# chenkovsky/aha

Measured on AMD Instinct MI355X. Metric: input GB/s scanned + M-hits/s, 100k-pattern AC over 1 GiB UTF-8 corpus, higher is better.
Workload: dtype u8

## Files before the change

aha_amd/csrc/image.hpp:

```cpp
#pragma once
#include <cstdint>

#include "../../include/aha_hip.h"

namespace aha {

struct DevAut {
  const void *slots;
  const int32_t *end_key;
  const uint32_t *end_info;
  const uint2 *key_ln;
  const uint32_t *key_cnt;
  const uint32_t *key_kc;
  const uint32_t *key_info;
  const uint2 *chain;
  const uint2 *chain_chars;
  uint32_t root;
  uint32_t n_slots;
  uint32_t max_len;
  uint32_t compact;
  uint32_t s1_lo;
  uint32_t s2_lo;
  uint32_t s2_hi;
  const uint32_t *stale_bits;
  const uint32_t *term_bits;
};

struct MatchArgs {
  const uint8_t *text;
  const uint64_t *doc_off;
  uint64_t n_docs;
  uint64_t n_bytes;
  uint64_t n_chunks;
  uint32_t chunk;
  int32_t chars;
  int32_t sep;
  uint32_t sep_block[8];
  int32_t has_nul;
  int32_t no_filter;
  int32_t no_pair;
  int32_t check_docs;
  uint32_t *counts;
  uint32_t *leads;
  uint64_t *blk_hits;
  uint64_t *blk_leads;
  uint64_t *docg;
  uint64_t *totals;
  aha_hit *out;
  uint64_t cap;
  uint64_t *doc_hit_off;
  int32_t count_only;
  unsigned long long *kc_visits;
  unsigned long long *kc_hits;
  unsigned long long *kc_out;
  int32_t neutral;
  uint32_t *cover_mask;
  uint64_t cover_bit0;
  int32_t cover_clear;
  int32_t fold;
};

constexpr int kBlock = 256;

constexpr int kV2Threads = 1024;
constexpr int kV2Piece = 32;
constexpr uint32_t kV2Slab = 512;
constexpr uint32_t kV2MaxS = 32768;

struct V2Args {
  const uint8_t *text;
  const uint64_t *doc_off;
  uint64_t n_docs;
  uint64_t n_bytes;
  uint64_t n_chunks;
  uint32_t S;
  uint32_t lds_slots;
  int32_t chars;
  int32_t sep;
  uint32_t sep_block[8];
  uint4 *ev;
  uint32_t *ev_aux;
  uint64_t ev_cap;
  unsigned long long *cursor;
  uint32_t *slab_used;
  uint32_t *ev_cnt;
  uint32_t *lead_cnt;
  uint32_t *chunk_doc0;
  uint32_t *doc_ev_rank;
  uint32_t *doc_lead_rank;
  uint64_t *ev_base;
  uint64_t *lead_base;
  uint64_t *blk_a;
  uint64_t *blk_b;
  uint4 *sorted_ev;
  uint32_t *sorted_aux;
  uint32_t *sorted_cnt;
  uint64_t *totals;
  int32_t direct;
  int32_t dense_hits;
  uint32_t ev_stride;
  uint2 *evd;
  uint32_t *evg;
  uint32_t *doc_hit_rank;
  uint32_t unit_bb;
  uint32_t *chunk_hits;
  uint64_t *hit_base;
  aha_hit *out;
  uint64_t cap;
  uint64_t *doc_hit_off;
  unsigned long long *publish;
  unsigned long long *clear_next;
  uint32_t doc_from, doc_lanes16;
};

struct UnitDev {
  const uint2 *slots;
  const uint32_t *root;
  const uint32_t *tables;
  uint32_t n_slots;
  uint32_t big_lo;
  uint32_t n_low;
  uint32_t g0;
  uint32_t base_bits;
  uint32_t n_syms;
  uint32_t max_len;
  uint32_t hdr_beside;
};
size_t unit_lds_bytes(uint32_t n_syms);
int unit_prepare(uint32_t n_syms);
void unit_launch_traverse(const UnitDev &U, const V2Args &M, uint32_t grid, void *stream);
void unit_launch_regroup(const DevAut &A, const V2Args &M, void *stream);
void unit_launch_expand(const uint2 *uend, const DevAut &A, const V2Args &M, uint32_t workgroups, void *stream);
void v2_launch_hit_scan(const V2Args &M, void *stream);
void v2_launch_lead_scan(const V2Args &M, void *stream);

struct SkipDev {
  const uint32_t *bloom;
  uint32_t log2;
  uint32_t k1;
};
int skip_prepare(uint32_t n_syms, uint32_t log2_words);
size_t skip_bitmap_bytes(uint64_t n_bytes);
void skip_launch_mark(const SkipDev &K, const V2Args &M, void *bitmap, uint32_t grid, void *stream);
void skip_launch_traverse(const UnitDev &U, const V2Args &M, const void *bitmap, uint32_t grid, void *stream);

struct PairDev {
  const uint32_t *bloom;
  const uint4 *tab;
  const uint8_t *disp;
  uint32_t bloom_log2, k1, log2, groups;
};

int pair_prepare(uint32_t n_syms, uint32_t bloom_log2, uint32_t groups);
uint32_t pair_tile_bytes();
size_t pair_cand_bytes(uint64_t cap);
size_t pair_walk_bytes(uint64_t cap);
void pair_launch(const PairDev &P, const UnitDev &U, const DevAut &A, const V2Args &M, void *tile_dn, void *cand, void *wres,
                 uint64_t cand_cap, uint32_t grid, void *mid_event, void *stream);

constexpr uint32_t kFilterMul = 0x9E3779B1u;
constexpr uint32_t kFilterLog2 = 14;
struct FilterDev {
  const uint32_t *bloom;
  uint32_t d;
  uint32_t log2;
};
bool filter_image_in_lds(uint32_t n_slots, uint32_t chunk_bytes, bool chars = false);
int filter_prepare();
size_t filter_chunk_rec_bytes();
void filter_launch_filter(const FilterDev &F, const V2Args &M, void *bitmap, void *chunk_rec, unsigned long long *non_ascii,
                          uint32_t cus, void *stream);
void filter_launch_walk(const DevAut &A, const V2Args &M, const void *bitmap, const void *chunk_rec, const unsigned long long *non_ascii,
                        uint32_t cus, void *stream);

void filter_launch_filter_fold(const FilterDev &F, const V2Args &M, void *bitmap, void *chunk_rec, unsigned long long *non_ascii,
                               uint32_t cus, void *stream);
void filter_launch_walk_fold(const DevAut &A, const V2Args &M, const void *bitmap, const void *chunk_rec,
                             const unsigned long long *non_ascii, uint32_t cus, void *stream);
void fold_launch_copy(const uint8_t *src, uint8_t *dst, uint64_t n_bytes, uint32_t max_blocks, void *stream);
void fold2_launch_copy(const uint8_t *src, uint8_t *dst, uint64_t n_bytes, const uint64_t *doc_offsets, uint64_t n_docs,
                       uint32_t max_blocks, void *stream);
void fold3_launch_copy(const uint8_t *src, uint8_t *dst, uint64_t n_bytes, const uint64_t *doc_offsets, uint64_t n_docs,
                       uint32_t max_blocks, void *stream);
void fold3_launch_fix(const uint8_t *src, uint8_t *dst, uint64_t n_bytes, const uint64_t *doc_offsets, uint64_t n_docs,
                      uint32_t max_blocks, void *stream);
uint32_t fold_grid(uint64_t n_bytes, uint32_t max_blocks);
void foldk_launch_copy(const uint8_t *src, uint8_t *dst, uint64_t n_bytes, const uint64_t *doc_offsets, uint64_t n_docs,
                       uint32_t max_blocks, void *stream);

size_t v2_lds_bytes(uint32_t lds_slots, bool compact);
int v2_prepare(bool compact, size_t lds_bytes);
void v2_launch_traverse(const DevAut &A, const V2Args &M, uint32_t grid, void *stream);
void v2_launch_chunk_scan(const V2Args &M, void *stream);
void v2_launch_sort(const DevAut &A, const V2Args &M, uint64_t n_records, void *stream);
void v2_launch_expand(const DevAut &A, const V2Args &M, uint64_t n_events, void *stream);
void v2_launch_direct_post(const DevAut &A, const V2Args &M, void *stream, void *ev_mid, bool counted = false);
void v2_launch_count_post(const DevAut &A, const V2Args &M, void *stream, bool counted);
void v2_launch_doc_offsets(const DevAut &A, const V2Args &M, void *stream);
void unit_launch_doc_offsets(const V2Args &M, void *stream);
void count_launch_visits(const DevAut &A, const V2Args &M, const uint2 *uend, unsigned long long *visits, uint32_t max_blocks,
                         void *stream);
void count_launch_chain(const uint2 *key_ln, uint32_t n_keys, const unsigned long long *visits, unsigned long long *out,
                        const unsigned long long *abortf, void *stream);

void cover_launch_clear(uint32_t *words, uint64_t n_words, const unsigned long long *abortf, uint32_t max_blocks, void *stream);
void cover_launch_spans(const DevAut &A, const V2Args &M, const uint2 *uend, uint64_t *cdoc, uint32_t *mask, uint64_t bit0,
                        uint32_t max_blocks, void *stream);
void cover_launch_redact(const uint8_t *src, uint8_t *dst, const uint32_t *mask, uint64_t n_bytes, uint8_t fill, uint32_t max_blocks,
                         void *stream);
void cover_launch_doc_covered(const uint32_t *mask, const uint64_t *doc_off, uint64_t n_docs, uint64_t *doc_covered,
                              uint32_t max_blocks, void *stream);
void cover_launch_total(const uint32_t *mask, uint64_t n_words, uint64_t *total, uint32_t max_blocks, void *stream);

struct DcItem {
  uint64_t begin;
  uint32_t *out;
  uint32_t n;
  uint32_t doc;
};
constexpr uint32_t kDcSortMax = 4096;
constexpr uint32_t kDcRangeKeys = 8192;
constexpr uint32_t kDcSliceHits = 1u << 16;
void doccount_launch_sort(const DcItem *items, uint32_t n_items, const void *hits, uint32_t *n_pairs, void *stream);
void doccount_launch_range(const DcItem *items, uint32_t n_items, const void *hits, uint32_t n_keys, uint32_t range_keys,
                           uint32_t *n_pairs, void *stream);
void doccount_launch_add(const DcItem *slices, uint32_t n_slices, const void *hits, uint32_t *rows, uint32_t n_keys,
                         uint32_t max_blocks, void *stream);
void doccount_launch_compact(const DcItem *docs, uint32_t n_rows, uint32_t *rows, uint32_t n_keys, uint32_t *n_pairs, void *stream);
void doccount_launch_compact64(const DcItem *doc, unsigned long long *row, uint32_t n_keys, uint32_t *n_pairs, void *stream);
void doccount_launch_gather(const uint64_t *pair_off, const uint32_t *const *src, uint64_t n_docs, uint64_t n, void *out,
                            void *stream);

uint64_t select_rank_blocks(uint64_t n_bytes);
void select_launch_longest(const void *hits, uint64_t n_hits, const uint64_t *hit_off, const uint64_t *rel, uint64_t nd, uint64_t nb,
                           uint64_t *L, uint32_t max_blocks, void *stream);
void select_launch_marks(const uint64_t *L, uint64_t nb, const uint64_t *rel, uint64_t nd, uint32_t *cover, uint32_t *doc_start,
                         uint32_t max_blocks, void *stream);
void select_launch_walk(const uint64_t *L, uint64_t nb, const uint32_t *cover, const uint32_t *doc_start, uint32_t *select,
                        uint32_t max_blocks, void *stream);
void select_launch_rank(const uint32_t *select, uint64_t nb, uint64_t *blk, uint32_t max_blocks, void *stream);
void select_launch_rank_docs(const uint32_t *select, const uint64_t *blk, const uint64_t *rel, uint64_t nd, uint64_t base,
                             uint64_t *out, uint32_t max_blocks, void *stream);
void select_launch_emit(const uint32_t *select, uint64_t nb, const uint64_t *blk, const uint64_t *L, const uint64_t *rel, uint64_t nd,
                        void *out, uint32_t max_blocks, void *stream);

void tokens_launch_spans(const uint64_t *L, uint64_t nb, const uint32_t *select, uint32_t *S, uint32_t max_blocks, void *stream);
void tokens_launch_starts(const uint8_t *text, uint64_t nb, const uint32_t *select, const uint32_t *S, const uint32_t *doc_start,
                          bool gap_runs, uint32_t *T, uint32_t max_blocks, void *stream);
void tokens_launch_emit(const uint32_t *T, uint64_t nb, const uint64_t *blk, const uint32_t *select, const uint32_t *doc_start,
                        const uint64_t *L, const uint64_t *rel, uint64_t nd, void *out, uint32_t max_blocks, void *stream);

struct RepEntry {
  uint64_t off;
  uint32_t len;
  uint32_t keep;
};
constexpr uint32_t kRpScanBlock = 256;
inline uint64_t replace_scan_blocks(uint64_t n) { return (n + kRpScanBlock - 1) / kRpScanBlock; }
void replace_launch_delta(const void *sel, uint64_t n, const uint64_t *dso, const uint64_t *doc_off, uint64_t n_docs,
                          const RepEntry *ent, uint32_t n_keys, uint64_t *start, int64_t *shift, uint32_t max_blocks, void *stream);
void replace_launch_scan(int64_t *shift, uint64_t n, int64_t *sums, uint32_t max_blocks, void *stream);
void replace_launch_doc_offsets(const uint64_t *doc_off, const uint64_t *dso, const int64_t *shift, uint64_t n_docs,
                                uint64_t *doc_out, uint32_t max_blocks, void *stream);
void replace_launch_copy(const uint8_t *text, const void *sel, const uint64_t *start, const int64_t *shift, uint64_t n,
                         const RepEntry *ent, uint32_t n_keys, const uint8_t *blob, uint8_t *out, uint64_t total,
                         uint32_t max_blocks, void *stream);

void grep_launch_ends(const uint8_t *corpus, uint64_t n_bytes, uint8_t delim, const uint64_t *doc_off, uint64_t n_docs, uint32_t *mask,
                      uint32_t max_blocks, void *stream);
void grep_launch_emit_ends(const uint32_t *mask, uint64_t n_bytes, const uint64_t *blk, uint64_t *rec_off, uint32_t max_blocks,
                           void *stream);
void grep_launch_flag(const uint64_t *dho, uint64_t n_docs, bool invert, uint32_t *keep, uint32_t *S, uint32_t *T, uint32_t max_blocks,
                      void *stream);
void grep_launch_runs(const uint32_t *S, const uint32_t *T, uint64_t n_docs, const uint64_t *blk_s, const uint64_t *blk_t,
                      const uint64_t *doc_off, uint64_t n_runs, uint64_t *start, int64_t *shift, void *sel, RepEntry *ent,
                      uint32_t max_blocks, void *stream);
void grep_launch_emit_docs(const uint32_t *keep, const uint32_t *S, uint64_t n_docs, const uint64_t *blk_k, const uint64_t *blk_s,
                           const uint64_t *doc_off, const int64_t *shift, uint64_t n_runs, uint64_t *kept_docs, uint64_t *doc_out,
                           uint32_t max_blocks, void *stream);

void excerpt_launch_edges(const uint32_t *M, uint64_t n_bytes, const uint64_t *doc_off, uint64_t n_docs, uint32_t *S, uint32_t *T,
                          uint32_t max_blocks, void *stream);
void excerpt_launch_windows(const uint32_t *S, const uint32_t *T, uint64_t n_bytes, const uint64_t *blk_s, const uint64_t *blk_t,
                            const uint8_t *corpus, const uint64_t *doc_off, uint64_t n_docs, uint32_t before, uint32_t after,
                            uint64_t n_runs, uint64_t *doc, uint64_t *w0, uint64_t *w1, uint32_t *first, uint32_t *last,
                            uint32_t max_blocks, void *stream);
void excerpt_launch_gaps(const uint32_t *first, const uint32_t *last, uint64_t n_runs, const uint64_t *blk_f, const uint64_t *blk_l,
                         const uint64_t *w0, const uint64_t *w1, uint64_t n_bytes, uint64_t n_exc, uint64_t *start, int64_t *shift,
                         void *sel, RepEntry *ent, uint32_t max_blocks, void *stream);
void excerpt_launch_emit(const uint64_t *start, const int64_t *shift, uint64_t n_exc, uint64_t *starts, uint64_t *out_off,
                         uint32_t max_blocks, void *stream);

constexpr uint32_t kRuleMaxTerms = 64;
constexpr uint32_t kRuleChunkClasses = 32;
void greprule_launch_keep(const uint32_t *rows, uint32_t n_classes, const uint64_t *doc_off, uint64_t n_docs,
                          const aha_rule_term *terms, uint32_t n_terms, bool invert, uint32_t *keep, uint32_t max_blocks, void *stream);
void greprule_launch_edges(const uint32_t *keep, uint64_t n_docs, uint32_t *S, uint32_t *T, uint32_t max_blocks, void *stream);

constexpr uint32_t kCcSlice = 2048;
constexpr uint32_t kCcTable = 8192;
void classcount_launch_add(const void *hits, uint64_t n_hits, const uint64_t *hit_off, uint64_t nd, const uint64_t *cls_off,
                           const uint32_t *cls_ids, uint32_t n_keys, uint32_t n_classes, uint32_t *out, uint32_t max_blocks,
                           void *stream);
void classcount_launch_fold_keys(const uint64_t *key_counts, uint32_t n_keys, const uint64_t *cls_off, const uint32_t *cls_ids,
                                 uint32_t *row, uint32_t max_blocks, void *stream);

void launch_hits_pack(const int32_t *hits, uint64_t n, int32_t *pairs, void *stream);
void launch_hits_unpack(const DevAut &A, const int32_t *pairs, uint64_t n, int chars, int32_t *hits, void *stream);
struct StreamFmt {
  uint32_t step_bits;
  uint32_t len_bits;
};
void launch_hits_pack4(const int32_t *hits, uint64_t n, uint32_t *stream_words, unsigned long long *n_words, StreamFmt F,
                       void *stream);
void launch_hits_unpack4(const DevAut &A, const uint32_t *stream_words, uint64_t n, int chars, int32_t *hits, StreamFmt F,
                         void *stream);
constexpr uint32_t kMaxSegs = 64;
void launch_hits_unpack4_segs(const DevAut &A, const uint32_t *land, const uint64_t *word_off, const uint64_t *n_hits,
                              const uint64_t *out_off, uint32_t n_segs, int chars, int32_t *hits, StreamFmt F, void *stream);

void launch_publish_words(const unsigned long long *src, unsigned long long *host_dst, int n, void *stream);
void launch_check_docs(const uint64_t *doc_off, uint64_t n_docs, uint64_t n_bytes, uint32_t *flag, unsigned long long *abort_word,
                       void *stream);

void launch_count(const DevAut &A, const MatchArgs &M, void *stream);
void launch_scan_blocks(const MatchArgs &M, uint64_t n_blocks, void *stream);
void launch_count_doc_offsets(const MatchArgs &M, void *stream);
void launch_docg(const MatchArgs &M, void *stream);
void launch_write(const DevAut &A, const MatchArgs &M, void *stream);
void launch_has_nul(const uint8_t *text, uint64_t n, uint64_t *flag, void *stream);
void launch_longest(const DevAut &A, const MatchArgs &M, int mode, bool write, void *stream);

}
```

aha_amd/csrc/scan_unit.hip:

```cpp
#include <hip/hip_runtime.h>

#include "automaton.hpp"
#include "devcommon.hpp"
#include "image.hpp"
#include "unit.hpp"

namespace aha {

namespace {

constexpr int kUPiece = 16;
constexpr int kUWin = 3 * kUPiece;
constexpr int kURow = kUWin + 4;
constexpr int kUWave = 64 * kURow;

__device__ __forceinline__ uint4 load16(const uint8_t *text, int64_t g, int64_t N) {
  uint4 v = make_uint4(0, 0, 0, 0);
  if (g >= 0 && g + 16 <= N) {
    v = *reinterpret_cast<const uint4 *>(text + g);
  } else if (g >= 0 && g < N) {
    uint32_t w0 = 0, w1 = 0, w2 = 0, w3 = 0;
#pragma unroll 1
    for (int j = 0; j < 16 && g + j < N; j++) {
      const uint32_t b = (uint32_t)text[g + j] << ((j & 3) * 8);
      w0 |= (j >> 2) == 0 ? b : 0u;
      w1 |= (j >> 2) == 1 ? b : 0u;
      w2 |= (j >> 2) == 2 ? b : 0u;
      w3 |= (j >> 2) == 3 ? b : 0u;
    }
    v = make_uint4(w0, w1, w2, w3);
  }
  return v;
}

__device__ __forceinline__ uint64_t wballot(bool p) { return __builtin_amdgcn_ballot_w64(p); }
__device__ __forceinline__ bool wany(bool p) { return __builtin_amdgcn_ballot_w64(p) != 0ull; }
__device__ __forceinline__ bool wall(bool p) { return __builtin_amdgcn_ballot_w64(!p) == 0ull; }

__host__ __device__ inline size_t u_lds_rows(uint32_t n_syms) {
  return (size_t)(kUTabWords + ((n_syms + 3u) & ~3u)) * 4 + (size_t)(kV2Threads / 64) * kUWave + 16;
}
__host__ __device__ inline size_t u_lds_prog(uint32_t n_syms) {
  return u_lds_rows(n_syms) + (size_t)(kV2Threads / 64) * 64 * 12;
}
__host__ __device__ inline size_t u_lds(uint32_t n_syms) {
  return u_lds_prog(n_syms) + (size_t)(kV2Threads / 64) * 4;
}

template <bool CHARS, int BB, bool HB>
__global__ __launch_bounds__(kV2Threads) void ku_traverse(UnitDev U, V2Args M) {
  extern __shared__ __attribute__((aligned(16))) uint8_t smem[];
  if (M.cursor[1] >= 16ull) return;
  uint32_t *tabw = reinterpret_cast<uint32_t *>(smem);
  uint32_t *rlw = tabw + kUTabWords;
  const uint32_t n_root = (U.n_syms + 3u) & ~3u;
  for (uint32_t i = threadIdx.x; i < kUTabWords; i += kV2Threads) tabw[i] = U.tables[i];
  for (uint32_t i = threadIdx.x; i < n_root; i += kV2Threads) rlw[i] = i < U.n_syms ? U.root[i] : 0u;
  uint32_t *prog = reinterpret_cast<uint32_t *>(smem + u_lds_prog(U.n_syms));
  if (threadIdx.x < kV2Threads / 64) prog[threadIdx.x] = 0u;
  __syncthreads();
  const uint32_t *rl = rlw;
  const uint4 *t0a = reinterpret_cast<const uint4 *>(tabw + kUT0a);
  const uint2 *t0b = reinterpret_cast<const uint2 *>(tabw + kUT0b);
  const uint8_t *tabb = reinterpret_cast<const uint8_t *>(tabw);
  uint8_t *in_base = smem + (size_t)(kUTabWords + n_root) * 4;
  const int lane = threadIdx.x & 63, wave = threadIdx.x >> 6;
  uint8_t *inl = in_base + wave * kUWave + lane * kURow;
  const uint32_t *row = reinterpret_cast<const uint32_t *>(inl);
  typedef uint32_t v3u __attribute__((ext_vector_type(3)));
  const uint32_t wbo = (uint32_t)u_lds_rows(U.n_syms) + (uint32_t)wave * (64u * 12u);
  const uint2 *slots = U.slots;
  const int64_t N = (int64_t)M.n_bytes;
  const uint64_t D = M.n_docs;
  const int64_t S = (int64_t)M.S;
  const int rounds = (int)(M.S / kUPiece);
  const int warm = U.max_len > 1 ? (int)U.max_len - 1 : 0;
  const int R = (warm + kUPiece - 1) / kUPiece;
  const uint32_t wave_u = (uint32_t)__builtin_amdgcn_readfirstlane(wave);
  uint32_t *my_prog = prog + (wave_u & 3u) * 4u + (wave_u >> 2);
  const uint4 *simd_prog = reinterpret_cast<const uint4 *>(prog + (wave_u & 3u) * 4u);
  uint32_t n_rounds = 0;

  const uint64_t n_tiles = (M.n_chunks + kV2Threads - 1) / kV2Threads;
  for (uint64_t tile = blockIdx.x; tile < n_tiles; tile += gridDim.x) {
    const uint64_t chunk = tile * kV2Threads + threadIdx.x;
    const uint32_t ev_stride = M.ev_stride;
    const bool live = chunk < M.n_chunks;
    const int64_t a = (int64_t)chunk * S;
    const int64_t e = live ? min(a + S, N) : a;
    uint64_t dn = 0;
    int64_t nb = INT64_MAX, doc_start = a, pos = e;
    uint32_t wfill = 0, wout = 0;
    const uint64_t wchunk0 = tile * kV2Threads + (uint64_t)wave * 64;
    uint32_t *wreg = M.evg + wchunk0 * M.ev_stride * 3;
    const uint32_t wcap = (uint32_t)min<uint64_t>(64, M.n_chunks > wchunk0 ? M.n_chunks - wchunk0 : 0) * M.ev_stride;
    uint32_t hits = 0;
    uint32_t lead_total = 0;
    uint32_t lc = 0, lc_exact = 0;
    uint32_t E = 0, seq = 0;
    uint32_t pc = 0;
    uint4 q1 = make_uint4(0, 0, 0, 0), q2 = q1, q3 = q1;
    uint32_t w[13] = {0, 0, 0, 0, 0, 0, 0, 0, 0, 0, 0, 0, 0};
    if (live) {
      dn = first_boundary(M.doc_off, D, (uint64_t)a);
      nb = (int64_t)M.doc_off[dn];
      pos = a;
      if (nb != a) {
        doc_start = (int64_t)M.doc_off[dn - 1];
        pos = a - min<int64_t>(a - doc_start, warm);
        if (CHARS) M.chunk_doc0[chunk] = (uint32_t)(dn - 1);
      } else if (CHARS) {
        M.chunk_doc0[chunk] = (uint32_t)dn;
      }
    }

    for (int r = -((R + 3) / 4) * 4 - 2; r <= rounds; r++) {
      {
        n_rounds++;
        if (lane == 0) *my_prog = n_rounds;
        const uint4 pm = *simd_prog;
        const uint32_t ahead = ((uint32_t)__builtin_amdgcn_readfirstlane(pm.x) > n_rounds) + ((uint32_t)__builtin_amdgcn_readfirstlane(pm.y) > n_rounds) +
                               ((uint32_t)__builtin_amdgcn_readfirstlane(pm.z) > n_rounds) + ((uint32_t)__builtin_amdgcn_readfirstlane(pm.w) > n_rounds);
        if (ahead == 0u)
          __builtin_amdgcn_s_setprio(0);
        else if (ahead == 1u)
          __builtin_amdgcn_s_setprio(1);
        else if (ahead == 2u)
          __builtin_amdgcn_s_setprio(2);
        else
          __builtin_amdgcn_s_setprio(3);
      }
      const int64_t pb = a + (int64_t)r * kUPiece;
      const int64_t pl = pb + 2 * kUPiece;
      const int64_t pend = min(pb + kUWin, e);
      {
        uint4 v;
        if ((pl & 63) == 0) {
          v = load16(M.text, pl, N);
          q1 = load16(M.text, pl + 16, N);
          q2 = load16(M.text, pl + 32, N);
          q3 = load16(M.text, pl + 48, N);
        } else {
          v = q1;
          q1 = q2;
          q2 = q3;
        }
#pragma unroll
        for (int i = 0; i < 9; i++) w[i] = w[i + 4];
        w[9] = v.x;
        w[10] = v.y;
        w[11] = v.z;
        w[12] = v.w;
        uint32_t *dst = reinterpret_cast<uint32_t *>(inl);
#pragma unroll
        for (int i = 0; i < 13; i++) dst[i] = w[i];
      }
      const bool need = live && pos < pend;
      if (!wany(need)) continue;
      uint32_t rel = kURow, lim = 0;
      if (need) {
        rel = (uint32_t)(pos - pb + 4);
        lim = (uint32_t)(pend - pb + 4);
      }
      uint32_t nb_rel = (nb >= pb - 4 && nb <= pb + kUWin) ? (uint32_t)(nb - pb + 4) : ~0u;
      const uint32_t n_rel = (N - pb) <= (int64_t)kUWin ? (uint32_t)max<int64_t>(N - pb + 4, 0) : ~0u;
      const int32_t a_rel = (int32_t)max<int64_t>(a - pb + 4, -128);
      const int32_t e_rel = (int32_t)min<int64_t>(e - pb + 4, 128);
      int32_t docrel = (int32_t)(pb - 4 - doc_start);

      for (;;) {
        const bool bnd = rel < lim && rel == nb_rel;
        if (wany(bnd)) {
          if (bnd) {
            const int64_t here = pb - 4 + rel;
            do {
              M.doc_ev_rank[dn] = seq;
              M.doc_hit_rank[dn] = hits;
              if (CHARS) M.doc_lead_rank[dn] = lead_total;
              dn++;
              nb = dn <= D ? (int64_t)M.doc_off[dn] : INT64_MAX;
            } while (nb == here);
            asm volatile("" : "+v"(nb));
            nb_rel = (nb <= pb + kUWin) ? (uint32_t)(nb - pb + 4) : ~0u;
            E = 0;
            pc = 0;
            lc = 0;
            lc_exact = 1;
            doc_start = here;
            docrel = -(int32_t)rel;
          }
        }
        uint32_t lim2 = min(lim, nb_rel);
        const uint32_t dend = min(nb_rel, n_rel);
        auto decode = [&](uint32_t at, uint32_t &o_code, uint32_t &o_L, bool &o_later) {
          const uint32_t lo = row[at >> 2], hi = row[(at >> 2) + 1];
          const uint32_t w4 = __builtin_amdgcn_alignbyte(hi, lo, at & 3u);
          const uint32_t b0 = w4 & 0xFFu;
          const uint4 q0 = t0a[b0];
          const uint2 q1 = t0b[b0];
          const uint32_t s1 = *reinterpret_cast<const uint32_t *>(tabb + q0.x + ((w4 >> 6) & 0x3FCu));
          const uint32_t s2 = *reinterpret_cast<const uint32_t *>(tabb + q0.y + ((w4 >> 14) & 0x3FCu));
          const uint32_t sum = q0.z + s1 + s2;
          const uint32_t want = q1.y;
          const bool in_doc = at + want <= dend;
          o_later = in_doc & at + want > (uint32_t)kURow;
          const bool whole = in_doc & sum < kUPoison;
          const bool o_good = whole & (sum - q0.w) < q1.x;
          o_L = whole ? want : 1u;
          if (CHARS) o_L |= (b0 & 0xC0u) != 0x80u ? 0x100u : 0u;
          o_code = o_good ? sum - kUBias : 0u;
        };
        uint32_t code, L;
        {
          bool later;
          decode(min(rel, (uint32_t)kURow), code, L, later);
          lim2 = later ? min(lim2, rel) : lim2;
          lim = later ? min(lim, rel) : lim;
        }
        bool all_left = false;
        for (;;) {
          const bool act = rel < lim2;
          all_left = wall(rel >= (uint32_t)(4 + kUPiece) || rel >= lim);
          if (all_left || !wany(act)) break;
          auto trip = [&]() -> uint32_t {
            uint32_t evc = 0;
            const bool good = code != 0u;
            const uint32_t Bq = u_child(E, BB);
            const bool hdr = u_hdr_pending(E);
            const bool grp = Bq >= U.big_lo & code >= U.n_low & !hdr;
            uint32_t se = grp ? (code >> 5) + U.g0 : code;
            se = hdr ? 0u : se;
            const uint32_t fc = BB == 22 ? (code & 7u) : min(code & 7u, 6u);
            const bool probe = act & good & (((E | 0x20000000u) >> ((uint32_t)BB + fc)) & 1u) != 0u & Bq != 0u;
            unsigned long long enw = 0;
            uint32_t hdw = 0;
            {
              const uint2 *ap = slots + (probe ? (Bq ^ se) : 0u);
              asm volatile("global_load_dwordx2 %0, %1, off" : "=v"(enw) : "v"(ap) : "memory");
              if (HB) {
                const uint2 *hp = slots + ((act & u_nfr(E) & !u_f1(E)) ? Bq : 0u);
                asm volatile("global_load_dword %0, %1, off" : "=v"(hdw) : "v"(hp) : "memory");
              }
            }
            if (act) {
              uint32_t n_code, n_L;
              bool n_later;
              const uint32_t Lb = CHARS ? (L & 0xFFu) : L;
              uint32_t rel_adv = rel + Lb;
              decode(rel_adv, n_code, n_L, n_later);
              const uint32_t rt = rl[code];
              const uint32_t rf = rl[pc];
              const bool viaroot0 = !u_nfr(E) | !good;
              const bool own0 = viaroot0 | u_f1(E);
              const uint32_t ft0 = u_f1(E) ? (rf & 0x7FFFFFFFu) : (Bq | u_all_filter(BB) | 0x20000000u);
              uint32_t miss0 = viaroot0 ? rt : (HB ? (rf & 0x7FFFFFFFu) : ft0);
              const uint32_t cb = code & 31u;
              uint32_t lowm = ~(~0u << cb);
              uint32_t gbit = (grp & probe) ? (1u << cb) : 0u;
              const bool pg = probe & !grp;
              const bool pgh = pg & !hdr;
              const int32_t last = (int32_t)rel_adv - 1;
              uint32_t wm = (last >= a_rel & last < e_rel) ? ~0u : 0u;
              uint32_t isl0 = (CHARS && (int32_t)rel >= a_rel) ? (L >> 8) : 0u;
              if (CHARS) asm volatile("" : "+v"(isl0));
              if (HB)
                asm volatile("s_waitcnt vmcnt(0)" : "+v"(enw), "+v"(hdw), "+v"(miss0), "+v"(rel_adv), "+v"(lowm), "+v"(gbit), "+v"(wm), "+v"(n_code), "+v"(n_L) : : "memory");
              else
                asm volatile("s_waitcnt vmcnt(0)" : "+v"(enw), "+v"(miss0), "+v"(rel_adv), "+v"(lowm), "+v"(gbit), "+v"(wm), "+v"(n_code), "+v"(n_L) : : "memory");
              const uint32_t enx = (uint32_t)enw, eny = (uint32_t)(enw >> 32);
              const bool symeq = u_sym(eny) == se;
              const bool symhit = symeq & pg;
              const bool hit = symeq & pgh;
              const bool redir = (enx & gbit) != 0u;
              const uint32_t rE = (__builtin_popcount(enx & lowm) + eny ^ code) | u_all_filter(BB);
              const bool viaroot = !(symhit | redir) & viaroot0;
              uint32_t missE = HB ? (own0 ? miss0 : hdw) : miss0;
              missE = redir ? rE : missE;
              E = symhit ? enx : missE;
              const bool consumed = hit | viaroot;
              const bool end = consumed & u_end(E);
              const uint32_t c4 = hit ? u_c4(eny) : 1u;
              pc = consumed ? code : pc;
              if (CHARS) {
                const uint32_t isl = consumed ? isl0 : 0u;
                lc += isl;
                lead_total += isl;
              }
              rel = consumed ? rel_adv : rel;
              const bool park = consumed & n_later;
              lim2 = park ? rel : lim2;
              lim = park ? rel : lim;
              code = consumed ? n_code : code;
              L = consumed ? n_L : L;
              evc = end ? (c4 & wm) : 0u;
            }
            return evc;
          };
          const uint32_t evc = trip();
          const uint64_t evm = wballot(evc != 0u);
          if (evm) {
            const bool ev = evc != 0u;
            const uint32_t kp = __popcll(evm);
            if (wfill + kp > 64u) {
              const uint32_t *q = reinterpret_cast<const uint32_t *>(smem + (wbo + __umul24((uint32_t)lane, 12u)));
              const v3u r = {q[0], q[1], q[2]};
              if ((uint32_t)lane < wfill && wout + (uint32_t)lane < wcap) *reinterpret_cast<v3u *>(wreg + (size_t)(wout + lane) * 3) = r;
              wout += wfill;
              wfill = 0;
            }
            const uint32_t my = wfill + __builtin_amdgcn_mbcnt_hi((uint32_t)(evm >> 32), __builtin_amdgcn_mbcnt_lo((uint32_t)evm, 0u));
            const uint32_t rx = u_rec_x(u_child(E, BB), (uint32_t)lane, evc, BB), rz = u_rec_z(hits, evc, BB);
            const uint32_t ry = CHARS ? ((lc << 1) | lc_exact) : (uint32_t)(docrel + (int32_t)rel);
            if (ev) {
              uint32_t *d = reinterpret_cast<uint32_t *>(smem + (wbo + __umul24(my, 12u)));
              d[0] = rx;
              d[1] = ry;
              d[2] = rz;
            }
            wfill += kp;
            seq += ev ? 1u : 0u;
            hits += evc;
          }
        }
        if (all_left || !wany(rel < lim)) break;
      }
      if (need) pos = pb - 4 + rel;
    }
    {
      const uint32_t *q = reinterpret_cast<const uint32_t *>(smem + (wbo + __umul24((uint32_t)lane, 12u)));
      const v3u r = {q[0], q[1], q[2]};
      if ((uint32_t)lane < wfill && wout + (uint32_t)lane < wcap) *reinterpret_cast<v3u *>(wreg + (size_t)(wout + lane) * 3) = r;
    }
    if (live) {
      M.ev_cnt[chunk] = seq;
      if (seq > ev_stride) M.cursor[1] = 2ull;
      if (CHARS) M.lead_cnt[chunk] = lead_total;
      M.chunk_hits[chunk] = hits;
      if (e == N) {
        while (dn <= D) {
          M.doc_ev_rank[dn] = seq;
          M.doc_hit_rank[dn] = hits;
          if (CHARS) M.doc_lead_rank[dn] = lead_total;
          dn++;
        }
      }
    }
  }
}

constexpr int kRgThreads = 256, kRgPer = 4, kRgBlock = kRgThreads * kRgPer, kRgSubs = kRgBlock / 64;
__global__ __launch_bounds__(kRgThreads) void ku_regroup(DevAut A, V2Args M) {
  __shared__ uint2 s_sorted[kRgBlock];
  __shared__ uint8_t s_lane[kRgBlock];
  __shared__ uint32_t s_cnt[kRgSubs][64], s_part[kRgThreads / 64][64];
  __shared__ uint32_t s_start[64], s_tot[64], s_run[64], s_hits[64];
  if (M.cursor[1]) return;
  const int lane = threadIdx.x & 63, wv = threadIdx.x >> 6;
  const uint64_t n_groups = (M.n_chunks + 63) / 64;
  const uint32_t stride = M.ev_stride;
  const uint32_t bb = M.unit_bb, bmask = (1u << bb) - 1u;
  for (uint64_t g = blockIdx.x; g < n_groups; g += gridDim.x) {
    __syncthreads();
    if (wv == 0) {
      s_run[lane] = 0;
      s_hits[lane] = 0;
    }
    const uint64_t c = g * 64 + lane;
    uint32_t total = c < M.n_chunks ? min(M.ev_cnt[c], stride) : 0u;
#pragma unroll
    for (int d = 32; d >= 1; d >>= 1) total += __shfl_xor(total, d, 64);
    const uint32_t *src = M.evg + g * 64 * stride * 3;
    uint2 *dst = M.evd + g * 64 * stride;
    uint2 nxt[kRgPer];
    uint32_t xn[kRgPer];
#pragma unroll
    for (int q = 0; q < kRgPer; q++) {
      const uint32_t i = q * kRgThreads + threadIdx.x;
      nxt[q] = i < total ? make_uint2(src[(size_t)i * 3], src[(size_t)i * 3 + 1]) : make_uint2(0, 0);
    }
#pragma unroll
    for (int q = 0; q < kRgPer; q++) xn[q] = (uint32_t)(q * kRgThreads) + threadIdx.x < total ? A.end_info[nxt[q].x & bmask] : 0u;
    for (uint32_t i0 = 0; i0 < total; i0 += kRgBlock) {
      uint2 rec[kRgPer];
      uint32_t x[kRgPer], rank[kRgPer], l[kRgPer];
      bool live[kRgPer];
#pragma unroll
      for (int q = 0; q < kRgPer; q++) {
        const uint32_t i = i0 + q * kRgThreads + threadIdx.x;
        live[q] = i < total;
        rec[q] = nxt[q];
        x[q] = xn[q];
        nxt[q] = i + kRgBlock < total ? make_uint2(src[(size_t)(i + kRgBlock) * 3], src[(size_t)(i + kRgBlock) * 3 + 1])
                                      : make_uint2(0, 0);
      }
#pragma unroll
      for (int q = 0; q < kRgPer; q++) {
        l[q] = (rec[q].x >> bb) & 63u;
        uint64_t same = __ballot(live[q]), mine = same;
#pragma unroll
        for (int b = 0; b < 6; b++) {
          const uint64_t bal = __ballot(live[q] & ((l[q] >> b) & 1u) != 0u);
          same &= ((l[q] >> b) & 1u) ? bal : ~bal;
          mine &= ((lane >> b) & 1) ? bal : ~bal;
        }
        rank[q] = __popcll(same & ((1ull << lane) - 1ull));
        s_cnt[q * (kRgThreads / 64) + wv][lane] = __popcll(mine);
      }
      __syncthreads();
      {
        uint32_t acc = 0;
#pragma unroll
        for (int r = 0; r < kRgSubs / (kRgThreads / 64); r++) {
          const uint32_t v = s_cnt[wv * (kRgSubs / (kRgThreads / 64)) + r][lane];
          s_cnt[wv * (kRgSubs / (kRgThreads / 64)) + r][lane] = acc;
          acc += v;
        }
        s_part[wv][lane] = acc;
      }
      __syncthreads();
      if (wv == 0) {
        uint32_t acc = 0;
#pragma unroll
        for (int w2 = 0; w2 < kRgThreads / 64; w2++) {
          const uint32_t v = s_part[w2][lane];
          s_part[w2][lane] = acc;
          acc += v;
        }
        s_tot[lane] = acc;
        s_start[lane] = wave_incl_scan(acc) - acc;
      }
      __syncthreads();
#pragma unroll
      for (int q = 0; q < kRgPer; q++) {
        if (live[q]) {
          const uint32_t sb = q * (kRgThreads / 64) + wv;
          const uint32_t p = s_start[l[q]] + s_part[sb / (kRgSubs / (kRgThreads / 64))][l[q]] + s_cnt[sb][l[q]] + rank[q];
          uint32_t cnt = x[q] >> 24;
          if (cnt == 255u) cnt = A.key_cnt[A.chain ? A.chain[x[q] & 0xFFFFFFu].y : (x[q] & 0xFFFFFFu)];
          s_sorted[p] = make_uint2(x[q], rec[q].y);
          s_lane[p] = (uint8_t)l[q];
          if (cnt) atomicAdd(&s_hits[l[q]], cnt);
        }
      }
      __syncthreads();
#pragma unroll
      for (int q = 0; q < kRgPer; q++)
        xn[q] = i0 + kRgBlock + (uint32_t)(q * kRgThreads) + threadIdx.x < total ? A.end_info[nxt[q].x & bmask] : 0u;
#pragma unroll
      for (int q = 0; q < kRgPer; q++) asm volatile("" : "+v"(xn[q]));
      const uint32_t nb = min(total - i0, (uint32_t)kRgBlock);
#pragma unroll
      for (int q = 0; q < kRgPer; q++) {
        const uint32_t p = q * kRgThreads + threadIdx.x;
        if (p < nb) {
          const uint32_t lp = s_lane[p];
          const uint32_t at = s_run[lp] + (p - s_start[lp]);
          if (at < stride) dst[(uint64_t)lp * stride + at] = s_sorted[p];
        }
      }
      __syncthreads();
      if (wv == 0) s_run[lane] += s_tot[lane];
    }
    __syncthreads();
    if (wv == 0 && c < M.n_chunks) M.chunk_hits[c] = s_hits[lane];
  }
}

constexpr int kXgThreads = 1024, kXgPer = 1, kXgBlock = kXgThreads * kXgPer, kXgStage = 1536;
constexpr int kXgCacheBits = 11;
template <bool CHARS>
__global__ __launch_bounds__(kXgThreads) void ku_expand_groups(const uint2 *uend, DevAut A, V2Args M) {
  __shared__ uint32_t s_hs[kXgStage], s_he[kXgStage], s_hk[kXgStage];
  __shared__ uint8_t s_hl[kXgStage];
  __shared__ uint32_t s_tot[2][64], s_start[64], s_run[64], s_all;
  __shared__ uint64_t s_base[64];
  __shared__ uint32_t s_adj[64];
  __shared__ unsigned long long s_cache[1 << kXgCacheBits];
  if (M.cursor[1]) return;
  const int lane = threadIdx.x & 63, wv = threadIdx.x >> 6;
  const uint64_t n_groups = (M.n_chunks + 63) / 64;
  const uint32_t stride = M.ev_stride;
  const uint32_t bb = M.unit_bb, bmask = (1u << bb) - 1u;
  for (uint32_t i = threadIdx.x; i < (1u << kXgCacheBits); i += kXgThreads) s_cache[i] = 0ull;
  for (uint64_t g = blockIdx.x; g < n_groups; g += gridDim.x) {
    __syncthreads();
    const uint64_t c = g * 64 + lane;
    if (wv == 0) {
      if (CHARS && c < M.n_chunks) s_adj[lane] = M.lead_cnt[c];
      s_base[lane] = c < M.n_chunks ? M.hit_base[c] : 0ull;
      s_run[lane] = 0;
      s_tot[0][lane] = 0;
    }
    uint32_t total = c < M.n_chunks ? min(M.ev_cnt[c], stride) : 0u;
#pragma unroll
    for (int d = 32; d >= 1; d >>= 1) total += __shfl_xor(total, d, 64);
    const uint32_t *src = M.evg + g * 64 * stride * 3;
    typedef uint32_t v3u __attribute__((ext_vector_type(3)));
    v3u nxt[kXgPer];
#pragma unroll
    for (int q = 0; q < kXgPer; q++) {
      const uint32_t i = q * kXgThreads + threadIdx.x;
      nxt[q] = i < total ? __builtin_nontemporal_load(reinterpret_cast<const v3u *>(src + (size_t)i * 3)) : v3u{0, 0, 0};
    }
    __syncthreads();
    uint32_t par = 0;
    for (uint32_t i0 = 0; i0 < total; i0 += kXgBlock, par ^= 1u) {
      v3u rec[kXgPer];
      uint2 ue[kXgPer];
      bool live[kXgPer], keep[kXgPer];
      uint32_t cs[kXgPer];
#pragma unroll
      for (int q = 0; q < kXgPer; q++) {
        const uint32_t i = i0 + q * kXgThreads + threadIdx.x;
        live[q] = i < total;
        rec[q] = nxt[q];
        nxt[q] = i + kXgBlock < total ? __builtin_nontemporal_load(reinterpret_cast<const v3u *>(src + (size_t)(i + kXgBlock) * 3)) : v3u{0, 0, 0};
        const uint32_t b = rec[q].x & bmask, n = u_rec_n(rec[q].x, rec[q].z, bb);
        cs[q] = (b * 0x9E3779B1u) >> (32 - kXgCacheBits);
        const unsigned long long ce = s_cache[cs[q]];
        const bool cached = live[q] & n == 1u & (uint32_t)ce == b + 1u;
        ue[q] = make_uint2((uint32_t)(ce >> 32), 0u);
        if (live[q] && !cached) ue[q] = uend[b];
        keep[q] = live[q] & !cached & n == 1u;
        if (live[q]) atomicAdd(&s_tot[par][(rec[q].x >> bb) & 63u], n);
      }
      __syncthreads();
      if (wv == 0) {
        const uint32_t t = s_tot[par][lane];
        const uint32_t incl = wave_incl_scan(t);
        s_start[lane] = incl - t;
        if (lane == 63) s_all = incl;
        s_tot[par ^ 1u][lane] = 0;
      }
      __syncthreads();
      const uint32_t T = s_all;
#pragma unroll
      for (int q = 0; q < kXgPer; q++)
        if (keep[q] && (ue[q].y >> 24) == 0u)
          atomicExch(&s_cache[cs[q]], (unsigned long long)ue[q].x << 32 | ((rec[q].x & bmask) + 1u));
      for (uint32_t w0 = 0; w0 < T; w0 += kXgStage) {
#pragma unroll
        for (int q = 0; q < kXgPer; q++) {
          if (live[q]) {
            const uint32_t l = (rec[q].x >> bb) & 63u, n = u_rec_n(rec[q].x, rec[q].z, bb);
            const uint32_t pos = s_start[l] + (u_rec_before(rec[q].z) - s_run[l]);
            const uint32_t end = CHARS ? (rec[q].y >> 1) + ((rec[q].y & 1u) ? 0u : s_adj[l]) : rec[q].y, co = ue[q].y & 0xFFFFFFu;
            uint32_t len = (ue[q].x >> 24) | (ue[q].y >> 24) << 8, key = ue[q].x & 0xFFFFFFu;
            for (uint32_t k = 0;;) {
              const uint32_t j = pos + k - w0;
              if (j < (uint32_t)kXgStage) {
                s_hs[j] = end - len;
                s_he[j] = end;
                s_hk[j] = key;
                s_hl[j] = (uint8_t)l;
              }
              if (++k >= n) break;
              const uint2 ce = (CHARS ? A.chain_chars : A.chain)[co + k];
              len = ce.x;
              key = ce.y;
            }
          }
        }
        __syncthreads();
        const uint32_t nh = min(T - w0, (uint32_t)kXgStage);
        for (uint32_t j = threadIdx.x; j < nh; j += kXgThreads) {
          const uint32_t l = s_hl[j];
          const uint64_t idx = s_base[l] + s_run[l] + (w0 + j - s_start[l]);
          if (idx < M.cap) {
            aha_hit hit;
            hit.start = (int32_t)s_hs[j];
            hit.end = (int32_t)s_he[j];
            hit.value = (int32_t)s_hk[j];
            M.out[idx] = hit;
          }
        }
        __syncthreads();
      }
      if (wv == 0) s_run[lane] += s_tot[par][lane];
    }
  }
}

__global__ __launch_bounds__(256) void ku_chunk_adj(V2Args M) {
  if (M.cursor[1]) return;
  const uint64_t c = (uint64_t)blockIdx.x * 256 + threadIdx.x;
  if (c >= M.n_chunks) return;
  const uint32_t d0 = M.chunk_doc0[c];
  const uint64_t dchunk = M.doc_off[d0] / M.S;
  M.lead_cnt[c] = (uint32_t)(M.lead_base[c] - (M.lead_base[dchunk] + M.doc_lead_rank[d0]));
}

__global__ __launch_bounds__(256) void ku_doc_offsets(V2Args M) {
  if (M.publish && blockIdx.x == 0 && threadIdx.x < 5) M.publish[threadIdx.x] = M.cursor[threadIdx.x];
  if (M.clear_next && blockIdx.x == 0 && threadIdx.x < 16) M.clear_next[threadIdx.x] = 0ull;
  if (M.cursor[1] || !M.doc_hit_off) return;
  const uint64_t d = (uint64_t)blockIdx.x * 256 + threadIdx.x;
  if (d > M.n_docs) return;
  const uint64_t q = M.doc_off[d];
  M.doc_hit_off[d] = q < M.n_bytes ? M.hit_base[q / M.S] + M.doc_hit_rank[d] : M.totals[0];
}

}

size_t unit_lds_bytes(uint32_t n_syms) { return u_lds(n_syms); }

int unit_prepare(uint32_t n_syms) {
  const int lds = (int)unit_lds_bytes(n_syms);
  int e = 0;
#define AHA_PREP_KU(C, B, H) \
  if (!e) e = (int)hipFuncSetAttribute((const void *)ku_traverse<C, B, H>, hipFuncAttributeMaxDynamicSharedMemorySize, lds);
  AHA_PREP_KU(false, 22, false) AHA_PREP_KU(true, 22, false) AHA_PREP_KU(false, 23, false) AHA_PREP_KU(true, 23, false)
  AHA_PREP_KU(false, 22, true) AHA_PREP_KU(true, 22, true) AHA_PREP_KU(false, 23, true) AHA_PREP_KU(true, 23, true)
#undef AHA_PREP_KU
  return e;
}

void unit_launch_traverse(const UnitDev &U, const V2Args &M, uint32_t grid, void *stream) {
  const size_t lds = unit_lds_bytes(U.n_syms);
#define AHA_LAUNCH_KU(C, B, H) hipLaunchKernelGGL((ku_traverse<C, B, H>), dim3(grid), dim3(kV2Threads), lds, (hipStream_t)stream, U, M)
#define AHA_LAUNCH_KU2(C, B) \
  do {                       \
    if (U.hdr_beside)        \
      AHA_LAUNCH_KU(C, B, true);  \
    else                     \
      AHA_LAUNCH_KU(C, B, false); \
  } while (0)
  if (U.base_bits == 23) {
    if (M.chars) AHA_LAUNCH_KU2(true, 23); else AHA_LAUNCH_KU2(false, 23);
  } else {
    if (M.chars) AHA_LAUNCH_KU2(true, 22); else AHA_LAUNCH_KU2(false, 22);
  }
#undef AHA_LAUNCH_KU2
#undef AHA_LAUNCH_KU
}

void unit_launch_doc_offsets(const V2Args &M, void *stream) {
  if (M.doc_hit_off)
    hipLaunchKernelGGL(ku_doc_offsets, dim3((uint32_t)((M.n_docs + 1 + 255) / 256)), dim3(256), 0, (hipStream_t)stream, M);
}

void unit_launch_regroup(const DevAut &A, const V2Args &M, void *stream) {
  const uint64_t n_groups = (M.n_chunks + 63) / 64;
  hipLaunchKernelGGL(ku_regroup, dim3((uint32_t)std::min<uint64_t>(n_groups, 1u << 16)), dim3(kRgThreads), 0,
                     (hipStream_t)stream, A, M);
}

void unit_launch_expand(const uint2 *uend, const DevAut &A, const V2Args &M, uint32_t workgroups, void *stream) {
  const uint64_t n_groups = (M.n_chunks + 63) / 64;
  const dim3 grid((uint32_t)std::max<uint64_t>(1, std::min<uint64_t>(n_groups, workgroups)));
  if (M.chars) {
    hipLaunchKernelGGL(ku_chunk_adj, dim3((uint32_t)((M.n_chunks + 255) / 256)), dim3(256), 0, (hipStream_t)stream, M);
    hipLaunchKernelGGL(ku_expand_groups<true>, grid, dim3(kXgThreads), 0, (hipStream_t)stream, uend, A, M);
  } else {
    hipLaunchKernelGGL(ku_expand_groups<false>, grid, dim3(kXgThreads), 0, (hipStream_t)stream, uend, A, M);
  }
  if (M.doc_hit_off)
    hipLaunchKernelGGL(ku_doc_offsets, dim3((uint32_t)((M.n_docs + 1 + 255) / 256)), dim3(256), 0, (hipStream_t)stream, M);
}

}
```

aha_amd/csrc/unit.cpp:

```cpp
#include "unit.hpp"

#include <algorithm>
#include <cstdio>
#include <cstdlib>
#include <cstring>
#include <chrono>

namespace aha {

namespace {

struct UTrans {
  uint32_t sym;
  uint32_t child;
  uint32_t raw;
};

}

static void build_unit_bits(const Automaton &a, UnitImage &u, bool force, uint32_t base_bits) {
  u = UnitImage();
  u.base_bits = base_bits;
  const uint32_t max_slots = 1u << base_bits;
  const uint32_t S = a.n_states;
  if (a.n_keys == 0 || S < 2) {
    u.why = "no keys";
    return;
  }
  if (a.n_keys > (1u << 24)) {
    u.why = "more than 2^24 keys";
    return;
  }
  std::vector<uint8_t> need(S, 0);
  for (uint32_t s = 0; s < S; s++) {
    for (uint32_t j = 0; j < a.n_child[s]; j++) {
      const uint32_t c = a.first_child[s] + j;
      const uint32_t b = a.in_label[c];
      if (need[s]) {
        if ((b & 0xC0u) != 0x80u) {
          u.why = "a key holds a lead byte without its continuation bytes";
          return;
        }
        need[c] = (uint8_t)(need[s] - 1);
      } else if (b < 0x80u) {
        need[c] = 0;
      } else if ((b & 0xE0u) == 0xC0u) {
        need[c] = 1;
      } else if ((b & 0xF0u) == 0xE0u) {
        need[c] = 2;
      } else {
        u.why = "a key holds a stray continuation byte or a byte >= 0xF0";
        return;
      }
    }
    if (a.key_of[s] >= 0 && need[s]) {
      u.why = "a key ends inside a unit";
      return;
    }
  }
  for (uint32_t s = 1; s < S; s++)
    if (need[s] == 0 && need[a.fail[s]] != 0) {
      u.why = "a fail link leaves the unit boundaries";
      return;
    }
  uint64_t multi = 0, all = 0;
  for (uint32_t s = 1; s < S; s++) {
    all++;
    if (a.in_label[s] >= 0x80u) multi++;
  }
  u.multi_permille = (uint32_t)(multi * 1000 / std::max<uint64_t>(all, 1));
  if (!force && u.multi_permille < 300) {
    u.why = "fewer than 30 % of the key bytes lie in multi-byte units";
    return;
  }

  std::vector<uint32_t> first(S + 1, 0);
  std::vector<UTrans> tr;
  tr.reserve(S);
  std::vector<uint32_t> ustates;
  uint32_t lo2 = ~0u, hi2 = 0, lo3 = ~0u, hi3 = 0;
  for (uint32_t s = 0; s < S; s++) {
    first[s] = (uint32_t)tr.size();
    if (need[s]) continue;
    ustates.push_back(s);
    for (uint32_t j = 0; j < a.n_child[s]; j++) {
      const uint32_t c1 = a.first_child[s] + j;
      const uint32_t b0 = a.in_label[c1];
      if (need[c1] == 0) {
        tr.push_back({(1u << 16) | b0, c1, b0});
        continue;
      }
      for (uint32_t j2 = 0; j2 < a.n_child[c1]; j2++) {
        const uint32_t c2 = a.first_child[c1] + j2;
        const uint32_t b1 = a.in_label[c2];
        if (need[c2] == 0) {
          const uint32_t p = ((b0 & 0x1Fu) << 6) | (b1 & 0x3Fu);
          lo2 = std::min(lo2, p);
          hi2 = std::max(hi2, p + 1);
          tr.push_back({(2u << 16) | p, c2, b0 | b1 << 8});
          continue;
        }
        for (uint32_t j3 = 0; j3 < a.n_child[c2]; j3++) {
          const uint32_t c3 = a.first_child[c2] + j3;
          const uint32_t b2 = a.in_label[c3];
          const uint32_t p = ((b0 & 0x0Fu) << 12) | ((b1 & 0x3Fu) << 6) | (b2 & 0x3Fu);
          lo3 = std::min(lo3, p);
          hi3 = std::max(hi3, p + 1);
          tr.push_back({(3u << 16) | p, c3, b0 | b1 << 8 | b2 << 16});
        }
      }
    }
  }
  first[S] = (uint32_t)tr.size();
  u.n_states = (uint32_t)ustates.size();
  u.n_trans = (uint32_t)tr.size();
  if (getenv("AHA_DEBUG")) fprintf(stderr, "aha: unit image: %u states, %u transitions, %u-bit bases\n", u.n_states, u.n_trans, base_bits);
  if ((uint64_t)u.n_states + u.n_states / 8 + 1 > max_slots) {
    u.why = "more states than the bases address";
    return;
  }

  u.c2lo = hi2 ? lo2 : 0;
  u.w2 = hi2 ? hi2 - lo2 : 0;
  u.c3lo = hi3 ? lo3 : 0;
  u.w3 = hi3 ? hi3 - lo3 : 0;
  u.n1 = 128;
  u.n2 = 129 + u.w2;
  u.n_syms = u.n2 + 1 + u.w3;
  if (u.n_syms > kUMaxSyms) {
    u.why = "the keys' characters span more symbols than the root table holds in LDS";
    return;
  }
  for (UTrans &t : tr) {
    const uint32_t cls = t.sym >> 16, p = t.sym & 0xFFFFu;
    t.sym = cls == 1 ? p : (cls == 2 ? 129 + (p - u.c2lo) : u.n2 + 1 + (p - u.c3lo));
  }
  for (uint32_t s : ustates)
    if (!std::is_sorted(tr.begin() + first[s], tr.begin() + first[s + 1], [](const UTrans &x, const UTrans &y) { return x.sym < y.sym; }))
      std::sort(tr.begin() + first[s], tr.begin() + first[s + 1], [](const UTrans &x, const UTrans &y) { return x.sym < y.sym; });
  u.tables.assign(kUTabWords, 0u);
  for (uint32_t b = 0; b < 256; b++) {
    uint32_t a1 = 0, a2 = 0, L = 1, lo = 1, span = 127;
    int64_t base = 0;
    if (b >= 1 && b < 0x80) {
      base = b;
    } else if ((b & 0xE0u) == 0xC0u) {
      L = 2;
      a1 = (kUA1 + 256) * 4;
      lo = 129;
      span = u.w2;
      base = 129 + (int64_t)((b & 0x1Fu) << 6) - u.c2lo;
    } else if ((b & 0xF0u) == 0xE0u) {
      L = 3;
      a1 = (kUA1 + 512) * 4;
      a2 = (kUA2 + 256) * 4;
      lo = u.n2 + 1;
      span = u.w3;
      base = (int64_t)u.n2 + 1 + (int64_t)((b & 0x0Fu) << 12) - u.c3lo;
    }
    if (L == 1) {
      a1 = kUA1 * 4;
      a2 = kUA2 * 4;
    } else if (L == 2) {
      a2 = kUA2 * 4;
    }
    u.tables[kUT0a + 4 * b + 0] = a1;
    u.tables[kUT0a + 4 * b + 1] = a2;
    u.tables[kUT0a + 4 * b + 2] = (uint32_t)(base + kUBias);
    u.tables[kUT0a + 4 * b + 3] = lo + kUBias;
    u.tables[kUT0b + 2 * b + 0] = span;
    u.tables[kUT0b + 2 * b + 1] = L;
    const bool cont = (b & 0xC0u) == 0x80u;
    u.tables[kUA1 + 256 + b] = cont ? (b & 0x3Fu) : kUPoison;
    u.tables[kUA1 + 512 + b] = cont ? ((b & 0x3Fu) << 6) : kUPoison;
    u.tables[kUA2 + 256 + b] = cont ? (b & 0x3Fu) : kUPoison;
  }

  std::vector<uint8_t> udepth(S, 0);
  for (uint32_t s : ustates)
    for (uint32_t t = first[s]; t < first[s + 1]; t++) udepth[tr[t].child] = (uint8_t)std::min<uint32_t>(udepth[s] + 1u, 255u);
  for (uint32_t s : ustates)
    if (udepth[s] == 1 && a.key_of[s] >= 0) u.unit_key = true;
  {
    std::vector<uint8_t> de(S, 0);
    for (uint32_t s : ustates)
      for (uint32_t t = first[s]; t < first[s + 1]; t++) {
        const uint32_t c = tr[t].child;
        de[c] = (uint8_t)std::min<uint32_t>(de[s] + ((udepth[c] >= 3 && a.key_of[c] >= 0) ? 1u : 0u), 255u);
        u.deep_ends_max = std::max<uint32_t>(u.deep_ends_max, de[c]);
      }
  }
  if (!u.unit_key) {
    struct Pair {
      uint32_t raw0, raw1, child, h;
    };
    std::vector<Pair> pairs;
    for (uint32_t t0 = first[0]; t0 < first[1]; t0++) {
      const uint32_t c0 = tr[t0].child;
      for (uint32_t t1 = first[c0]; t1 < first[c0 + 1]; t1++) pairs.push_back({tr[t0].raw, tr[t1].raw, tr[t1].child, 0u});
    }
    u.n_pairs = (uint32_t)pairs.size();
    static const uint32_t k1s[] = {kSkipKA, 0xC2B2AFu, 0x27D4EBu, 0x165667u, 0xD3A264u, 0xFD7047u, 0xB55A4Fu, 0x7FEB35u};
    bool placed = false;
    for (uint32_t k1 : k1s) {
      if (pairs.empty() || pairs.size() > (size_t)kPairMaxGroups * 8) break;
      for (Pair &p : pairs) p.h = sk_hash(sk_part(p.raw0), p.raw1, k1);
      std::vector<uint32_t> sorted(pairs.size());
      for (size_t i = 0; i < pairs.size(); i++) sorted[i] = pairs[i].h;
      std::sort(sorted.begin(), sorted.end());
      if (std::adjacent_find(sorted.begin(), sorted.end()) != sorted.end()) continue;
      uint32_t G = 256;
      while (G < kPairMaxGroups && G * 4u < pairs.size()) G <<= 1;
      std::vector<std::vector<uint32_t>> groups(G);
      for (uint32_t i = 0; i < pairs.size(); i++) groups[pt_group(pairs[i].h, G)].push_back(i);
      std::vector<uint32_t> order(G);
      for (uint32_t g = 0; g < G; g++) order[g] = g;
      std::stable_sort(order.begin(), order.end(), [&](uint32_t x, uint32_t y) { return groups[x].size() > groups[y].size(); });
      uint32_t lg = 8;
      while (((size_t)1 << lg) * 2u < pairs.size() * 3u) lg++;
      for (; lg <= 21 && !placed; lg++) {
        std::vector<uint32_t> tab((size_t)4 << lg, 0u);
        std::vector<uint8_t> disp(G, 0);
        bool okp = true;
        std::vector<uint32_t> slots;
        for (uint32_t gi = 0; okp && gi < G; gi++) {
          const std::vector<uint32_t> &grp = groups[order[gi]];
          if (grp.empty()) break;
          uint32_t d = 0;
          for (; d < 256; d++) {
            slots.clear();
            bool fits = true;
            for (uint32_t i : grp) {
              const uint32_t sl = pt_slot(pairs[i].h, d, lg);
              if (tab[4 * (size_t)sl] != 0 || std::find(slots.begin(), slots.end(), sl) != slots.end()) {
                fits = false;
                break;
              }
              slots.push_back(sl);
            }
            if (fits) break;
          }
          if (d == 256) {
            okp = false;
            break;
          }
          disp[order[gi]] = (uint8_t)d;
          for (size_t j = 0; j < grp.size(); j++) {
            const Pair &p = pairs[grp[j]];
            uint32_t cf = 0;
            for (uint32_t t2 = first[p.child]; t2 < first[p.child + 1]; t2++) cf |= pt_cls(tr[t2].raw);
            const int32_t key = a.key_of[p.child];
            const uint32_t c4 = key >= 0 ? std::min<uint32_t>(a.key_cnt[key], kUMaxC4) : 0u;
            uint32_t *e = &tab[4 * (size_t)slots[j]];
            e[0] = p.raw0 | c4 << 24;
            e[1] = p.raw1;
            e[2] = (uint32_t)key;
            e[3] = cf;
          }
        }
        if (okp) {
          u.pair_tab.swap(tab);
          u.pair_disp.swap(disp);
          u.pair_log2 = lg;
          u.pair_groups = G;
          u.pair_k1 = k1;
          placed = true;
        }
      }
      if (placed) break;
    }
    if (!placed) {
      u.pair_k1 = kSkipKA;
      for (Pair &p : pairs) p.h = sk_hash(sk_part(p.raw0), p.raw1, u.pair_k1);
    }
    for (uint32_t lg = kSkipMinLog2; !pairs.empty() && lg <= kSkipMaxLog2; lg++) {
      u.mark_bloom.assign((size_t)1 << lg, 0u);
      for (const Pair &p : pairs) u.mark_bloom[sk_word(p.h, lg)] |= sk_mask(p.h);
      uint64_t bits = 0;
      for (uint32_t x : u.mark_bloom) bits += (uint64_t)__builtin_popcount(x);
      u.mark_log2 = lg;
      u.mark_fill_permille = (uint32_t)(bits * 1000 / ((uint64_t)32 << lg));
      if (bits * 16 <= ((uint64_t)32 << lg)) break;
    }
  }
  auto has_header = [&](uint32_t s) {
    return s != 0 && a.fail[s] != 0 && udepth[a.fail[s]] != 1;
  };

  u.n_low = std::min<uint32_t>((u.n2 + 1 + 31u) & ~31u, 512u);
  u.g0 = u.n_low - (u.n_low >> 5);
  const uint32_t n_groups = u.n_syms > u.n_low ? (u.n_syms - u.n_low + 31u) / 32u : 0u;
  uint32_t bb = 64;
  while (bb < u.n_low + n_groups) bb <<= 1;
  u.big_block = bb;
  constexpr uint32_t kBlk = 1u << 15;
  constexpr uint32_t kMaxBlocks = kUMaxSlots / kBlk;
  struct Bits {
    std::vector<uint64_t> w;
    explicit Bits(size_t n) : w((n + 63) / 64, 0ull) {}
    bool get(uint32_t i) const { return (w[i >> 6] >> (i & 63)) & 1ull; }
    void set(uint32_t i) { w[i >> 6] |= 1ull << (i & 63); }
  };
  Bits used(kUMaxSlots), isb(kUMaxSlots);
  std::vector<uint32_t> freec(kMaxBlocks, kBlk), curw(kMaxBlocks, 0);
  std::vector<uint32_t> idfree(kMaxBlocks, kBlk);
  std::vector<uint32_t> base(S, 0);
  used.set(0);
  isb.set(0);
  freec[0]--;
  idfree[0]--;
  uint32_t n_open = 1, n_big = 0, n_bases = 1;
  std::vector<uint32_t> order, bigs;
  for (uint32_t s : ustates) {
    if (s == 0) continue;
    const uint32_t deg = first[s + 1] - first[s];
    if (deg >= kUBigDegree) {
      bigs.push_back(s);
    } else if (deg + (has_header(s) ? 1u : 0u) > 0) {
      order.push_back(s);
    }
  }
  n_big = (uint32_t)bigs.size();
  auto nsym = [&](uint32_t s) { return first[s + 1] - first[s] + (has_header(s) ? 1u : 0u); };
  std::stable_sort(order.begin(), order.end(), [&](uint32_t x, uint32_t y) {
    const uint32_t cx = udepth[x] == 1 ? 0u : 1u, cy = udepth[y] == 1 ? 0u : 1u;
    if (cx != cy) return cx < cy;
    return nsym(x) > nsym(y);
  });
  auto open_block = [&]() -> bool {
    if ((uint64_t)(n_open + 1) * kBlk + (uint64_t)n_big * bb > max_slots) {
      if (getenv("AHA_DEBUG"))
        fprintf(stderr, "aha: unit image: %u blocks open, %u big states of %u slots, %u bases so far: no room for another block\n",
                n_open, n_big, bb, n_bases);
      return false;
    }
    n_open++;
    return true;
  };
  uint32_t sy[kUBigDegree + 1];
  auto try_block = [&](uint32_t blk, uint32_t k) -> uint32_t {
    const uint32_t fr = freec[blk];
    if (fr < k) return 0;
    uint64_t budget = fr;
    if ((double)fr * idfree[blk] / kBlk < 0.5) return 0;
    if (k > 1) {
      double p = (double)idfree[blk] / kBlk;
      const double fl = (double)fr / kBlk;
      for (uint32_t i = 1; i < k; i++) p *= fl;
      if (p * fr < 0.5) return 0;
      budget = std::min<uint64_t>(fr, (uint64_t)(4.0 / p) + 1024);
    }
    const uint32_t w0 = blk * (kBlk / 64), nw = kBlk / 64;
    uint32_t wi = curw[blk];
    for (uint32_t step = 0; step < nw && budget; step++, wi = wi + 1 < nw ? wi + 1 : 0) {
      uint64_t fw = ~used.w[w0 + wi];
      while (fw && budget) {
        const uint32_t f = ((w0 + wi) << 6) + (uint32_t)__builtin_ctzll(fw);
        fw &= fw - 1;
        budget--;
        const uint32_t cand = f ^ sy[0];
        if (cand == 0 || isb.get(cand)) continue;
        bool okc = true;
        for (uint32_t i = 1; okc && i < k; i++) okc = !used.get(cand ^ sy[i]);
        if (okc) {
          curw[blk] = wi;
          return cand;
        }
      }
    }
    return 0;
  };
  uint32_t lowest = 0;
  std::vector<uint32_t> dead(kMaxBlocks, ~0u);
  auto place = [&](uint32_t k) -> uint32_t {
    while (lowest < n_open && freec[lowest] == 0) lowest++;
    for (uint32_t blk = lowest;; blk++) {
      if (blk == n_open && !open_block()) return 0;
      if (k >= dead[blk]) continue;
      const uint32_t b = try_block(blk, k);
      if (!b && (k > 1 || (double)freec[blk] * idfree[blk] / kBlk < 8.0)) dead[blk] = k;
      if (b) {
        for (uint32_t i = 0; i < k; i++) used.set(b ^ sy[i]);
        freec[blk] -= k;
        isb.set(b);
        idfree[blk]--;
        n_bases++;
        return b;
      }
    }
  };
  std::vector<std::vector<uint32_t>> big_runs(n_big);
  auto place_runs = [&]() -> bool {
    uint32_t t = kBlk;
    for (uint32_t bi = 0; bi < n_big; bi++) {
      const uint32_t s = bigs[bi];
      big_runs[bi].assign(n_groups, 0u);
      for (uint32_t q = first[s]; q < first[s + 1];) {
        if (tr[q].sym < u.n_low) {
          q++;
          continue;
        }
        const uint32_t g = (tr[q].sym - u.n_low) >> 5;
        uint32_t q2 = q;
        while (q2 < first[s + 1] && ((tr[q2].sym - u.n_low) >> 5) == g) q2++;
        const uint32_t cnt = q2 - q;
        for (;; t++) {
          if (t + cnt > n_open * kBlk) {
            if (!open_block()) return false;
          }
          if ((t & (kBlk - 1)) + cnt > kBlk) {
            t = (t | (kBlk - 1));
            continue;
          }
          bool okr = true;
          for (uint32_t j = 0; okr && j < cnt; j++) okr = !used.get(t + j) && !isb.get((t + j) ^ tr[q + j].sym);
          if (okr) break;
        }
        for (uint32_t j = 0; j < cnt; j++) {
          used.set(t + j);
          if (!isb.get((t + j) ^ tr[q + j].sym)) {
            isb.set((t + j) ^ tr[q + j].sym);
            idfree[t / kBlk]--;
            n_bases++;
          }
        }
        freec[t / kBlk] -= cnt;
        big_runs[bi][g] = t;
        t += cnt;
        q = q2;
      }
    }
    return true;
  };
  bool runs_done = n_big == 0 || n_groups == 0;
  const auto t_place = std::chrono::steady_clock::now();
  auto lap = [&](const char *what) {
    if (getenv("AHA_DEBUG"))
      fprintf(stderr, "aha: unit image: %s at %.2f s, %u blocks\n", what,
              std::chrono::duration<double>(std::chrono::steady_clock::now() - t_place).count(), n_open);
  };
  for (size_t oi = 0; oi < order.size(); oi++) {
    const uint32_t s = order[oi];
    if (!runs_done && udepth[s] != 1) {
      if (!place_runs()) {
        u.why = "more transitions than the bases address";
        return;
      }
      runs_done = true;
    }
    uint32_t k = 0;
    for (uint32_t t = first[s]; t < first[s + 1]; t++) sy[k++] = tr[t].sym;
    if (has_header(s)) sy[k++] = 0u;
    const uint32_t b = place(k);
    if (!b) {
      u.why = "more transitions than the bases address";
      return;
    }
    base[s] = b;
  }
  if (!runs_done && !place_runs()) {
    u.why = "more transitions than the bases address";
    return;
  }
  lap("states with slots placed");
  {
    uint32_t n_ids = 0;
    for (uint32_t s : ustates)
      if (s != 0 && first[s + 1] == first[s] && !has_header(s)) n_ids++;
    while ((uint64_t)n_open * kBlk < (uint64_t)n_bases + n_ids + 1)
      if (!open_block()) {
        u.why = "more states than the bases address";
        return;
      }
    uint32_t idc = 1;
    for (uint32_t s : ustates) {
      if (s == 0 || first[s + 1] != first[s] || has_header(s)) continue;
      while (isb.get(idc)) idc++;
      base[s] = idc;
      isb.set(idc);
    }
  }
  const uint32_t n_shared = n_open * kBlk;
  const uint32_t n_slots = ((n_shared + n_big * bb) + kBlk - 1) & ~(kBlk - 1);
  for (uint32_t bi = 0; bi < n_big; bi++) base[bigs[bi]] = n_shared + bi * bb;

  auto word = [&](uint32_t st) -> uint32_t {
    uint32_t flt = 0;
    for (uint32_t q = first[st]; q < first[st + 1]; q++) flt |= 1u << (tr[q].sym & 7u);
    if (first[st + 1] - first[st] >= kUBigDegree) flt = 0xFFu;
    const bool nfr = a.fail[st] != 0, f1 = nfr && udepth[a.fail[st]] == 1;
    return base[st] | ((flt << base_bits) & u_all_filter(base_bits)) | (f1 ? (1u << 29) : 0u) | (nfr ? (1u << 30) : 0u) |
           (a.key_of[st] >= 0 ? 0x80000000u : 0u);
  };
  auto u_c4_of = [](const Automaton &au, uint32_t st) -> uint32_t {
    return au.key_of[st] >= 0 ? std::min<uint32_t>(au.key_cnt[au.key_of[st]], kUMaxC4) : 0u;
  };
  u.n_slots = n_slots;
  u.n_shared = n_shared;
  u.n_big = n_big;
  u.slots.assign(n_slots, 0ull);
  u.end_key.assign(n_slots, -1);
  u.root.assign(u.n_syms, 0u);
  std::vector<uint32_t> big_index(n_big ? S : 0, 0u);
  for (uint32_t bi = 0; bi < n_big; bi++) big_index[bigs[bi]] = bi;
  for (uint32_t s : ustates) {
    const uint32_t b = base[s];
    const bool big = s != 0 && first[s + 1] - first[s] >= kUBigDegree;
    if (has_header(s)) {
      u.slots[b] = (uint64_t)(word(a.fail[s]) & 0x7FFFFFFFu);
      u.n_nfr++;
    }
    if (a.key_of[s] >= 0) u.end_key[b] = a.key_of[s];
    for (uint32_t t = first[s]; t < first[s + 1]; t++) {
      const uint32_t c = tr[t].child, sym = tr[t].sym;
      const uint64_t entry = ((uint64_t)(sym | u_c4_of(a, c) << 16) << 32) | word(c);
      if (s == 0) {
        u.root[sym] = word(c);
      } else if (!big || sym < u.n_low) {
        u.slots[b ^ sym] = entry;
      } else {
        const uint32_t g = (sym - u.n_low) >> 5, run = big_runs[big_index[s]][g];
        uint64_t &rec = u.slots[b + u.n_low + g];
        const uint32_t bits = (uint32_t)rec, rank = (uint32_t)__builtin_popcount(bits);
        rec = ((uint64_t)run << 32) | (bits | 1u << ((sym - u.n_low) & 31u));
        u.slots[run + rank] = entry;
      }
    }
  }
  u.ok = true;
}

void build_unit(const Automaton &a, UnitImage &u, bool force) {
  const char *bw = getenv("AHA_UNIT_BASE_BITS");
  if (bw && strcmp(bw, "23") == 0) {
    build_unit_bits(a, u, force, 23u);
    return;
  }
  build_unit_bits(a, u, force, 22u);
  if (!u.ok && strstr(u.why, "bases address")) build_unit_bits(a, u, force, 23u);
}

}
```

aha_amd/csrc/unit.hpp:

```cpp
#pragma once

#include <cstdint>
#include <vector>

#include "automaton.hpp"

namespace aha {

constexpr uint32_t kUMaxSlots = 1u << 23;
constexpr uint32_t kUBigDegree = 48;
constexpr uint32_t kUMaxSyms = 21756;
constexpr uint32_t kUBias = 1u << 17;
constexpr uint32_t kUPoison = 1u << 24;
constexpr uint32_t kUT0a = 0, kUT0b = 1024, kUA1 = 1536, kUA2 = 2304, kUTabWords = 2816;

AHA_HD inline uint32_t u_child(uint32_t lo, uint32_t bb = 22u) { return lo & ((1u << bb) - 1u); }
AHA_HD inline uint32_t u_all_filter(uint32_t bb) { return ((1u << (29u - bb)) - 1u) << bb; }
constexpr uint32_t kUMaxC4 = 255u;
constexpr uint32_t kUFusedMaxChain = 15u;
AHA_HD inline uint32_t u_rec_x(uint32_t base, uint32_t lane, uint32_t n, uint32_t bb) {
  return base | lane << bb | (n & ((1u << (26u - bb)) - 1u)) << (bb + 6u);
}
AHA_HD inline uint32_t u_rec_z(uint32_t hits_before, uint32_t n, uint32_t bb) { return hits_before | (n >> (26u - bb)) << 27; }
AHA_HD inline uint32_t u_rec_n(uint32_t x, uint32_t z, uint32_t bb) { return (x >> (bb + 6u)) | (z >> 27) << (26u - bb); }
AHA_HD inline uint32_t u_rec_before(uint32_t z) { return z & 0x7FFFFFFu; }
AHA_HD inline bool u_f1(uint32_t lo) { return ((lo >> 29) & 1u) != 0; }
AHA_HD inline bool u_nfr(uint32_t lo) { return ((lo >> 30) & 1u) != 0; }
AHA_HD inline bool u_end(uint32_t lo) { return (lo >> 31) != 0; }
AHA_HD inline uint32_t u_sym(uint32_t hi) { return hi & 0xFFFFu; }
AHA_HD inline uint32_t u_c4(uint32_t hi) { return (hi >> 16) & 255u; }
AHA_HD inline bool u_hdr_pending(uint32_t lo) { return ((lo >> 29) & 3u) == 1u; }

constexpr uint32_t kSkipKA = 0x9E3779u, kSkipKB = 0x85EBCBu;
constexpr uint32_t kSkipMinLog2 = 10, kSkipMaxLog2 = 14;
AHA_HD inline uint32_t sk_mul24(uint32_t a, uint32_t b) { return (a & 0xFFFFFFu) * (b & 0xFFFFFFu); }
AHA_HD inline uint32_t sk_part(uint32_t c0) {
  const uint32_t g = sk_mul24(c0, kSkipKB);
  return (g >> 11) | (g << 21);
}
AHA_HD inline uint32_t sk_hash(uint32_t part, uint32_t c1, uint32_t k1 = kSkipKA) {
  const uint32_t h = sk_mul24(c1, k1) + part;
  return h ^ (h >> 16);
}
AHA_HD inline uint32_t sk_word(uint32_t h, uint32_t log2_words) { return h >> (32u - log2_words); }
AHA_HD inline uint32_t sk_mask(uint32_t h) { return (1u << (h & 31u)) | (1u << ((h >> 5) & 31u)); }

constexpr uint32_t kPairMix = 0x2545F491u, kPairKC = 0xC2B2AFu;
constexpr uint32_t kPairMaxGroups = 16384;
constexpr uint32_t kPairMaxDeepEnds = 3;
AHA_HD inline uint32_t pt_group(uint32_t h, uint32_t n_groups) { return (h >> 7) & (n_groups - 1u); }
AHA_HD inline uint32_t pt_slot(uint32_t h, uint32_t d, uint32_t log2_slots) {
  const uint32_t t = h * kPairMix;
  return ((t >> (32u - log2_slots)) + d * ((t << 1) | 1u)) & ((1u << log2_slots) - 1u);
}
AHA_HD inline uint32_t pt_cls(uint32_t raw) {
  const uint32_t g = sk_mul24(raw, kPairKC);
  return (1u << (g >> 27)) | (1u << ((g >> 22) & 31u));
}

struct UnitImage {
  bool ok = false;
  const char *why = "";
  uint32_t n_slots = 0;
  uint32_t n_shared = 0;
  uint32_t n_big = 0, big_block = 0;
  uint32_t n_low = 0, g0 = 0;
  uint32_t base_bits = 22;
  std::vector<uint64_t> slots;
  std::vector<int32_t> end_key;
  std::vector<uint32_t> root;
  std::vector<uint32_t> tables;
  uint32_t n_syms = 0;
  uint32_t n1 = 128, n2 = 0;
  uint32_t c2lo = 0, w2 = 0, c3lo = 0, w3 = 0;
  uint32_t n_states = 0, n_trans = 0, n_nfr = 0;
  uint32_t multi_permille = 0;
  std::vector<uint32_t> mark_bloom;
  uint32_t mark_log2 = 0;
  uint32_t n_pairs = 0;
  uint32_t mark_fill_permille = 0;
  bool unit_key = false;
  uint32_t pair_k1 = kSkipKA;
  std::vector<uint32_t> pair_tab;
  std::vector<uint8_t> pair_disp;
  uint32_t pair_log2 = 0, pair_groups = 0;
  uint32_t deep_ends_max = 0;
};

void build_unit(const Automaton &a, UnitImage &u, bool force = false);

}
```

Before: 494.8.

## Add 21-bit base encoding for unit automaton images with dedicated traverse kernel

Moves the traverse kernel into a shared header and adds a 21-bit-base variant, picked automatically when the slot table and identities fit in 2^21 and exceed a minimum size, unless skip/pair engines are opted in. Fewer base bits leave more filter bits in each state word (u_all_filter widens), so fewer transitions should need a global slot probe. The cost is extra build logic and another kernel instantiation. Correctness now depends on tracking the identity range accurately.

```diff
diff --git a/aha_amd/csrc/image.hpp b/aha_amd/csrc/image.hpp
--- a/aha_amd/csrc/image.hpp
+++ b/aha_amd/csrc/image.hpp
@@ -129,6 +129,8 @@
 size_t unit_lds_bytes(uint32_t n_syms);
 int unit_prepare(uint32_t n_syms);
 void unit_launch_traverse(const UnitDev &U, const V2Args &M, uint32_t grid, void *stream);
+int unit21_prepare(uint32_t n_syms);
+void unit21_launch_traverse(const UnitDev &U, const V2Args &M, uint32_t grid, void *stream);
 void unit_launch_regroup(const DevAut &A, const V2Args &M, void *stream);
 void unit_launch_expand(const uint2 *uend, const DevAut &A, const V2Args &M, uint32_t workgroups, void *stream);
 void v2_launch_hit_scan(const V2Args &M, void *stream);
diff --git a/aha_amd/csrc/scan_unit.hip b/aha_amd/csrc/scan_unit.hip
--- a/aha_amd/csrc/scan_unit.hip
+++ b/aha_amd/csrc/scan_unit.hip
@@ -1,352 +1,8 @@
-#include <hip/hip_runtime.h>
-
-#include "automaton.hpp"
-#include "devcommon.hpp"
-#include "image.hpp"
-#include "unit.hpp"
+#include "scan_unit_walk.hpp"
 
 namespace aha {
 
 namespace {
-
-constexpr int kUPiece = 16;
-constexpr int kUWin = 3 * kUPiece;
-constexpr int kURow = kUWin + 4;
-constexpr int kUWave = 64 * kURow;
-
-__device__ __forceinline__ uint4 load16(const uint8_t *text, int64_t g, int64_t N) {
-  uint4 v = make_uint4(0, 0, 0, 0);
-  if (g >= 0 && g + 16 <= N) {
-    v = *reinterpret_cast<const uint4 *>(text + g);
-  } else if (g >= 0 && g < N) {
-    uint32_t w0 = 0, w1 = 0, w2 = 0, w3 = 0;
-#pragma unroll 1
-    for (int j = 0; j < 16 && g + j < N; j++) {
-      const uint32_t b = (uint32_t)text[g + j] << ((j & 3) * 8);
-      w0 |= (j >> 2) == 0 ? b : 0u;
-      w1 |= (j >> 2) == 1 ? b : 0u;
-      w2 |= (j >> 2) == 2 ? b : 0u;
-      w3 |= (j >> 2) == 3 ? b : 0u;
-    }
-    v = make_uint4(w0, w1, w2, w3);
-  }
-  return v;
-}
-
-__device__ __forceinline__ uint64_t wballot(bool p) { return __builtin_amdgcn_ballot_w64(p); }
-__device__ __forceinline__ bool wany(bool p) { return __builtin_amdgcn_ballot_w64(p) != 0ull; }
-__device__ __forceinline__ bool wall(bool p) { return __builtin_amdgcn_ballot_w64(!p) == 0ull; }
-
-__host__ __device__ inline size_t u_lds_rows(uint32_t n_syms) {
-  return (size_t)(kUTabWords + ((n_syms + 3u) & ~3u)) * 4 + (size_t)(kV2Threads / 64) * kUWave + 16;
-}
-__host__ __device__ inline size_t u_lds_prog(uint32_t n_syms) {
-  return u_lds_rows(n_syms) + (size_t)(kV2Threads / 64) * 64 * 12;
-}
-__host__ __device__ inline size_t u_lds(uint32_t n_syms) {
-  return u_lds_prog(n_syms) + (size_t)(kV2Threads / 64) * 4;
-}
-
-template <bool CHARS, int BB, bool HB>
-__global__ __launch_bounds__(kV2Threads) void ku_traverse(UnitDev U, V2Args M) {
-  extern __shared__ __attribute__((aligned(16))) uint8_t smem[];
-  if (M.cursor[1] >= 16ull) return;
-  uint32_t *tabw = reinterpret_cast<uint32_t *>(smem);
-  uint32_t *rlw = tabw + kUTabWords;
-  const uint32_t n_root = (U.n_syms + 3u) & ~3u;
-  for (uint32_t i = threadIdx.x; i < kUTabWords; i += kV2Threads) tabw[i] = U.tables[i];
-  for (uint32_t i = threadIdx.x; i < n_root; i += kV2Threads) rlw[i] = i < U.n_syms ? U.root[i] : 0u;
-  uint32_t *prog = reinterpret_cast<uint32_t *>(smem + u_lds_prog(U.n_syms));
-  if (threadIdx.x < kV2Threads / 64) prog[threadIdx.x] = 0u;
-  __syncthreads();
-  const uint32_t *rl = rlw;
-  const uint4 *t0a = reinterpret_cast<const uint4 *>(tabw + kUT0a);
-  const uint2 *t0b = reinterpret_cast<const uint2 *>(tabw + kUT0b);
-  const uint8_t *tabb = reinterpret_cast<const uint8_t *>(tabw);
-  uint8_t *in_base = smem + (size_t)(kUTabWords + n_root) * 4;
-  const int lane = threadIdx.x & 63, wave = threadIdx.x >> 6;
-  uint8_t *inl = in_base + wave * kUWave + lane * kURow;
-  const uint32_t *row = reinterpret_cast<const uint32_t *>(inl);
-  typedef uint32_t v3u __attribute__((ext_vector_type(3)));
-  const uint32_t wbo = (uint32_t)u_lds_rows(U.n_syms) + (uint32_t)wave * (64u * 12u);
-  const uint2 *slots = U.slots;
-  const int64_t N = (int64_t)M.n_bytes;
-  const uint64_t D = M.n_docs;
-  const int64_t S = (int64_t)M.S;
-  const int rounds = (int)(M.S / kUPiece);
-  const int warm = U.max_len > 1 ? (int)U.max_len - 1 : 0;
-  const int R = (warm + kUPiece - 1) / kUPiece;
-  const uint32_t wave_u = (uint32_t)__builtin_amdgcn_readfirstlane(wave);
-  uint32_t *my_prog = prog + (wave_u & 3u) * 4u + (wave_u >> 2);
-  const uint4 *simd_prog = reinterpret_cast<const uint4 *>(prog + (wave_u & 3u) * 4u);
-  uint32_t n_rounds = 0;
-
-  const uint64_t n_tiles = (M.n_chunks + kV2Threads - 1) / kV2Threads;
-  for (uint64_t tile = blockIdx.x; tile < n_tiles; tile += gridDim.x) {
-    const uint64_t chunk = tile * kV2Threads + threadIdx.x;
-    const uint32_t ev_stride = M.ev_stride;
-    const bool live = chunk < M.n_chunks;
-    const int64_t a = (int64_t)chunk * S;
-    const int64_t e = live ? min(a + S, N) : a;
-    uint64_t dn = 0;
-    int64_t nb = INT64_MAX, doc_start = a, pos = e;
-    uint32_t wfill = 0, wout = 0;
-    const uint64_t wchunk0 = tile * kV2Threads + (uint64_t)wave * 64;
-    uint32_t *wreg = M.evg + wchunk0 * M.ev_stride * 3;
-    const uint32_t wcap = (uint32_t)min<uint64_t>(64, M.n_chunks > wchunk0 ? M.n_chunks - wchunk0 : 0) * M.ev_stride;
-    uint32_t hits = 0;
-    uint32_t lead_total = 0;
-    uint32_t lc = 0, lc_exact = 0;
-    uint32_t E = 0, seq = 0;
-    uint32_t pc = 0;
-    uint4 q1 = make_uint4(0, 0, 0, 0), q2 = q1, q3 = q1;
-    uint32_t w[13] = {0, 0, 0, 0, 0, 0, 0, 0, 0, 0, 0, 0, 0};
-    if (live) {
-      dn = first_boundary(M.doc_off, D, (uint64_t)a);
-      nb = (int64_t)M.doc_off[dn];
-      pos = a;
-      if (nb != a) {
-        doc_start = (int64_t)M.doc_off[dn - 1];
-        pos = a - min<int64_t>(a - doc_start, warm);
-        if (CHARS) M.chunk_doc0[chunk] = (uint32_t)(dn - 1);
-      } else if (CHARS) {
-        M.chunk_doc0[chunk] = (uint32_t)dn;
-      }
-    }
-
-    for (int r = -((R + 3) / 4) * 4 - 2; r <= rounds; r++) {
-      {
-        n_rounds++;
-        if (lane == 0) *my_prog = n_rounds;
-        const uint4 pm = *simd_prog;
-        const uint32_t ahead = ((uint32_t)__builtin_amdgcn_readfirstlane(pm.x) > n_rounds) + ((uint32_t)__builtin_amdgcn_readfirstlane(pm.y) > n_rounds) +
-                               ((uint32_t)__builtin_amdgcn_readfirstlane(pm.z) > n_rounds) + ((uint32_t)__builtin_amdgcn_readfirstlane(pm.w) > n_rounds);
-        if (ahead == 0u)
-          __builtin_amdgcn_s_setprio(0);
-        else if (ahead == 1u)
-          __builtin_amdgcn_s_setprio(1);
-        else if (ahead == 2u)
-          __builtin_amdgcn_s_setprio(2);
-        else
-          __builtin_amdgcn_s_setprio(3);
-      }
-      const int64_t pb = a + (int64_t)r * kUPiece;
-      const int64_t pl = pb + 2 * kUPiece;
-      const int64_t pend = min(pb + kUWin, e);
-      {
-        uint4 v;
-        if ((pl & 63) == 0) {
-          v = load16(M.text, pl, N);
-          q1 = load16(M.text, pl + 16, N);
-          q2 = load16(M.text, pl + 32, N);
-          q3 = load16(M.text, pl + 48, N);
-        } else {
-          v = q1;
-          q1 = q2;
-          q2 = q3;
-        }
-#pragma unroll
-        for (int i = 0; i < 9; i++) w[i] = w[i + 4];
-        w[9] = v.x;
-        w[10] = v.y;
-        w[11] = v.z;
-        w[12] = v.w;
-        uint32_t *dst = reinterpret_cast<uint32_t *>(inl);
-#pragma unroll
-        for (int i = 0; i < 13; i++) dst[i] = w[i];
-      }
-      const bool need = live && pos < pend;
-      if (!wany(need)) continue;
-      uint32_t rel = kURow, lim = 0;
-      if (need) {
-        rel = (uint32_t)(pos - pb + 4);
-        lim = (uint32_t)(pend - pb + 4);
-      }
-      uint32_t nb_rel = (nb >= pb - 4 && nb <= pb + kUWin) ? (uint32_t)(nb - pb + 4) : ~0u;
-      const uint32_t n_rel = (N - pb) <= (int64_t)kUWin ? (uint32_t)max<int64_t>(N - pb + 4, 0) : ~0u;
-      const int32_t a_rel = (int32_t)max<int64_t>(a - pb + 4, -128);
-      const int32_t e_rel = (int32_t)min<int64_t>(e - pb + 4, 128);
-      int32_t docrel = (int32_t)(pb - 4 - doc_start);
-
-      for (;;) {
-        const bool bnd = rel < lim && rel == nb_rel;
-        if (wany(bnd)) {
-          if (bnd) {
-            const int64_t here = pb - 4 + rel;
-            do {
-              M.doc_ev_rank[dn] = seq;
-              M.doc_hit_rank[dn] = hits;
-              if (CHARS) M.doc_lead_rank[dn] = lead_total;
-              dn++;
-              nb = dn <= D ? (int64_t)M.doc_off[dn] : INT64_MAX;
-            } while (nb == here);
-            asm volatile("" : "+v"(nb));
-            nb_rel = (nb <= pb + kUWin) ? (uint32_t)(nb - pb + 4) : ~0u;
-            E = 0;
-            pc = 0;
-            lc = 0;
-            lc_exact = 1;
-            doc_start = here;
-            docrel = -(int32_t)rel;
-          }
-        }
-        uint32_t lim2 = min(lim, nb_rel);
-        const uint32_t dend = min(nb_rel, n_rel);
-        auto decode = [&](uint32_t at, uint32_t &o_code, uint32_t &o_L, bool &o_later) {
-          const uint32_t lo = row[at >> 2], hi = row[(at >> 2) + 1];
-          const uint32_t w4 = __builtin_amdgcn_alignbyte(hi, lo, at & 3u);
-          const uint32_t b0 = w4 & 0xFFu;
-          const uint4 q0 = t0a[b0];
-          const uint2 q1 = t0b[b0];
-          const uint32_t s1 = *reinterpret_cast<const uint32_t *>(tabb + q0.x + ((w4 >> 6) & 0x3FCu));
-          const uint32_t s2 = *reinterpret_cast<const uint32_t *>(tabb + q0.y + ((w4 >> 14) & 0x3FCu));
-          const uint32_t sum = q0.z + s1 + s2;
-          const uint32_t want = q1.y;
-          const bool in_doc = at + want <= dend;
-          o_later = in_doc & at + want > (uint32_t)kURow;
-          const bool whole = in_doc & sum < kUPoison;
-          const bool o_good = whole & (sum - q0.w) < q1.x;
-          o_L = whole ? want : 1u;
-          if (CHARS) o_L |= (b0 & 0xC0u) != 0x80u ? 0x100u : 0u;
-          o_code = o_good ? sum - kUBias : 0u;
-        };
-        uint32_t code, L;
-        {
-          bool later;
-          decode(min(rel, (uint32_t)kURow), code, L, later);
-          lim2 = later ? min(lim2, rel) : lim2;
-          lim = later ? min(lim, rel) : lim;
-        }
-        bool all_left = false;
-        for (;;) {
-          const bool act = rel < lim2;
-          all_left = wall(rel >= (uint32_t)(4 + kUPiece) || rel >= lim);
-          if (all_left || !wany(act)) break;
-          auto trip = [&]() -> uint32_t {
-            uint32_t evc = 0;
-            const bool good = code != 0u;
-            const uint32_t Bq = u_child(E, BB);
-            const bool hdr = u_hdr_pending(E);
-            const bool grp = Bq >= U.big_lo & code >= U.n_low & !hdr;
-            uint32_t se = grp ? (code >> 5) + U.g0 : code;
-            se = hdr ? 0u : se;
-            const uint32_t fc = BB == 22 ? (code & 7u) : min(code & 7u, 6u);
-            const bool probe = act & good & (((E | 0x20000000u) >> ((uint32_t)BB + fc)) & 1u) != 0u & Bq != 0u;
-            unsigned long long enw = 0;
-            uint32_t hdw = 0;
-            {
-              const uint2 *ap = slots + (probe ? (Bq ^ se) : 0u);
-              asm volatile("global_load_dwordx2 %0, %1, off" : "=v"(enw) : "v"(ap) : "memory");
-              if (HB) {
-                const uint2 *hp = slots + ((act & u_nfr(E) & !u_f1(E)) ? Bq : 0u);
-                asm volatile("global_load_dword %0, %1, off" : "=v"(hdw) : "v"(hp) : "memory");
-              }
-            }
-            if (act) {
-              uint32_t n_code, n_L;
-              bool n_later;
-              const uint32_t Lb = CHARS ? (L & 0xFFu) : L;
-              uint32_t rel_adv = rel + Lb;
-              decode(rel_adv, n_code, n_L, n_later);
-              const uint32_t rt = rl[code];
-              const uint32_t rf = rl[pc];
-              const bool viaroot0 = !u_nfr(E) | !good;
-              const bool own0 = viaroot0 | u_f1(E);
-              const uint32_t ft0 = u_f1(E) ? (rf & 0x7FFFFFFFu) : (Bq | u_all_filter(BB) | 0x20000000u);
-              uint32_t miss0 = viaroot0 ? rt : (HB ? (rf & 0x7FFFFFFFu) : ft0);
-              const uint32_t cb = code & 31u;
-              uint32_t lowm = ~(~0u << cb);
-              uint32_t gbit = (grp & probe) ? (1u << cb) : 0u;
-              const bool pg = probe & !grp;
-              const bool pgh = pg & !hdr;
-              const int32_t last = (int32_t)rel_adv - 1;
-              uint32_t wm = (last >= a_rel & last < e_rel) ? ~0u : 0u;
-              uint32_t isl0 = (CHARS && (int32_t)rel >= a_rel) ? (L >> 8) : 0u;
-              if (CHARS) asm volatile("" : "+v"(isl0));
-              if (HB)
-                asm volatile("s_waitcnt vmcnt(0)" : "+v"(enw), "+v"(hdw), "+v"(miss0), "+v"(rel_adv), "+v"(lowm), "+v"(gbit), "+v"(wm), "+v"(n_code), "+v"(n_L) : : "memory");
-              else
-                asm volatile("s_waitcnt vmcnt(0)" : "+v"(enw), "+v"(miss0), "+v"(rel_adv), "+v"(lowm), "+v"(gbit), "+v"(wm), "+v"(n_code), "+v"(n_L) : : "memory");
-              const uint32_t enx = (uint32_t)enw, eny = (uint32_t)(enw >> 32);
-              const bool symeq = u_sym(eny) == se;
-              const bool symhit = symeq & pg;
-              const bool hit = symeq & pgh;
-              const bool redir = (enx & gbit) != 0u;
-              const uint32_t rE = (__builtin_popcount(enx & lowm) + eny ^ code) | u_all_filter(BB);
-              const bool viaroot = !(symhit | redir) & viaroot0;
-              uint32_t missE = HB ? (own0 ? miss0 : hdw) : miss0;
-              missE = redir ? rE : missE;
-              E = symhit ? enx : missE;
-              const bool consumed = hit | viaroot;
-              const bool end = consumed & u_end(E);
-              const uint32_t c4 = hit ? u_c4(eny) : 1u;
-              pc = consumed ? code : pc;
-              if (CHARS) {
-                const uint32_t isl = consumed ? isl0 : 0u;
-                lc += isl;
-                lead_total += isl;
-              }
-              rel = consumed ? rel_adv : rel;
-              const bool park = consumed & n_later;
-              lim2 = park ? rel : lim2;
-              lim = park ? rel : lim;
-              code = consumed ? n_code : code;
-              L = consumed ? n_L : L;
-              evc = end ? (c4 & wm) : 0u;
-            }
-            return evc;
-          };
-          const uint32_t evc = trip();
-          const uint64_t evm = wballot(evc != 0u);
-          if (evm) {
-            const bool ev = evc != 0u;
-            const uint32_t kp = __popcll(evm);
-            if (wfill + kp > 64u) {
-              const uint32_t *q = reinterpret_cast<const uint32_t *>(smem + (wbo + __umul24((uint32_t)lane, 12u)));
-              const v3u r = {q[0], q[1], q[2]};
-              if ((uint32_t)lane < wfill && wout + (uint32_t)lane < wcap) *reinterpret_cast<v3u *>(wreg + (size_t)(wout + lane) * 3) = r;
-              wout += wfill;
-              wfill = 0;
-            }
-            const uint32_t my = wfill + __builtin_amdgcn_mbcnt_hi((uint32_t)(evm >> 32), __builtin_amdgcn_mbcnt_lo((uint32_t)evm, 0u));
-            const uint32_t rx = u_rec_x(u_child(E, BB), (uint32_t)lane, evc, BB), rz = u_rec_z(hits, evc, BB);
-            const uint32_t ry = CHARS ? ((lc << 1) | lc_exact) : (uint32_t)(docrel + (int32_t)rel);
-            if (ev) {
-              uint32_t *d = reinterpret_cast<uint32_t *>(smem + (wbo + __umul24(my, 12u)));
-              d[0] = rx;
-              d[1] = ry;
-              d[2] = rz;
-            }
-            wfill += kp;
-            seq += ev ? 1u : 0u;
-            hits += evc;
-          }
-        }
-        if (all_left || !wany(rel < lim)) break;
-      }
-      if (need) pos = pb - 4 + rel;
-    }
-    {
-      const uint32_t *q = reinterpret_cast<const uint32_t *>(smem + (wbo + __umul24((uint32_t)lane, 12u)));
-      const v3u r = {q[0], q[1], q[2]};
-      if ((uint32_t)lane < wfill && wout + (uint32_t)lane < wcap) *reinterpret_cast<v3u *>(wreg + (size_t)(wout + lane) * 3) = r;
-    }
-    if (live) {
-      M.ev_cnt[chunk] = seq;
-      if (seq > ev_stride) M.cursor[1] = 2ull;
-      if (CHARS) M.lead_cnt[chunk] = lead_total;
-      M.chunk_hits[chunk] = hits;
-      if (e == N) {
-        while (dn <= D) {
-          M.doc_ev_rank[dn] = seq;
-          M.doc_hit_rank[dn] = hits;
-          if (CHARS) M.doc_lead_rank[dn] = lead_total;
-          dn++;
-        }
-      }
-    }
-  }
-}
 
 constexpr int kRgThreads = 256, kRgPer = 4, kRgBlock = kRgThreads * kRgPer, kRgSubs = kRgBlock / 64;
 __global__ __launch_bounds__(kRgThreads) void ku_regroup(DevAut A, V2Args M) {
@@ -612,7 +268,7 @@
   AHA_PREP_KU(false, 22, false) AHA_PREP_KU(true, 22, false) AHA_PREP_KU(false, 23, false) AHA_PREP_KU(true, 23, false)
   AHA_PREP_KU(false, 22, true) AHA_PREP_KU(true, 22, true) AHA_PREP_KU(false, 23, true) AHA_PREP_KU(true, 23, true)
 #undef AHA_PREP_KU
-  return e;
+  return e ? e : unit21_prepare(n_syms);
 }
 
 void unit_launch_traverse(const UnitDev &U, const V2Args &M, uint32_t grid, void *stream) {
@@ -625,7 +281,9 @@
     else                     \
       AHA_LAUNCH_KU(C, B, false); \
   } while (0)
-  if (U.base_bits == 23) {
+  if (U.base_bits == 21) {
+    unit21_launch_traverse(U, M, grid, stream);
+  } else if (U.base_bits == 23) {
     if (M.chars) AHA_LAUNCH_KU2(true, 23); else AHA_LAUNCH_KU2(false, 23);
   } else {
     if (M.chars) AHA_LAUNCH_KU2(true, 22); else AHA_LAUNCH_KU2(false, 22);
diff --git a/aha_amd/csrc/scan_unit21.hip b/aha_amd/csrc/scan_unit21.hip
--- /dev/null
+++ b/aha_amd/csrc/scan_unit21.hip
@@ -0,0 +1,26 @@
+#include "scan_unit_walk.hpp"
+
+namespace aha {
+
+int unit21_prepare(uint32_t n_syms) {
+  const int lds = (int)u_lds(n_syms);
+  int e = 0;
+#define AHA_PREP_KU(C, H) \
+  if (!e) e = (int)hipFuncSetAttribute((const void *)ku_traverse<C, 21, H>, hipFuncAttributeMaxDynamicSharedMemorySize, lds);
+  AHA_PREP_KU(false, false) AHA_PREP_KU(true, false) AHA_PREP_KU(false, true) AHA_PREP_KU(true, true)
+#undef AHA_PREP_KU
+  return e;
+}
+
+void unit21_launch_traverse(const UnitDev &U, const V2Args &M, uint32_t grid, void *stream) {
+  const size_t lds = u_lds(U.n_syms);
+#define AHA_LAUNCH_KU(C, H) hipLaunchKernelGGL((ku_traverse<C, 21, H>), dim3(grid), dim3(kV2Threads), lds, (hipStream_t)stream, U, M)
+  if (M.chars) {
+    if (U.hdr_beside) AHA_LAUNCH_KU(true, true); else AHA_LAUNCH_KU(true, false);
+  } else {
+    if (U.hdr_beside) AHA_LAUNCH_KU(false, true); else AHA_LAUNCH_KU(false, false);
+  }
+#undef AHA_LAUNCH_KU
+}
+
+}
diff --git a/aha_amd/csrc/scan_unit_walk.hpp b/aha_amd/csrc/scan_unit_walk.hpp
--- /dev/null
+++ b/aha_amd/csrc/scan_unit_walk.hpp
@@ -0,0 +1,356 @@
+#pragma once
+
+#include <hip/hip_runtime.h>
+
+#include "automaton.hpp"
+#include "devcommon.hpp"
+#include "image.hpp"
+#include "unit.hpp"
+
+namespace aha {
+
+namespace {
+
+constexpr int kUPiece = 16;
+constexpr int kUWin = 3 * kUPiece;
+constexpr int kURow = kUWin + 4;
+constexpr int kUWave = 64 * kURow;
+
+__device__ __forceinline__ uint4 load16(const uint8_t *text, int64_t g, int64_t N) {
+  uint4 v = make_uint4(0, 0, 0, 0);
+  if (g >= 0 && g + 16 <= N) {
+    v = *reinterpret_cast<const uint4 *>(text + g);
+  } else if (g >= 0 && g < N) {
+    uint32_t w0 = 0, w1 = 0, w2 = 0, w3 = 0;
+#pragma unroll 1
+    for (int j = 0; j < 16 && g + j < N; j++) {
+      const uint32_t b = (uint32_t)text[g + j] << ((j & 3) * 8);
+      w0 |= (j >> 2) == 0 ? b : 0u;
+      w1 |= (j >> 2) == 1 ? b : 0u;
+      w2 |= (j >> 2) == 2 ? b : 0u;
+      w3 |= (j >> 2) == 3 ? b : 0u;
+    }
+    v = make_uint4(w0, w1, w2, w3);
+  }
+  return v;
+}
+
+__device__ __forceinline__ uint64_t wballot(bool p) { return __builtin_amdgcn_ballot_w64(p); }
+__device__ __forceinline__ bool wany(bool p) { return __builtin_amdgcn_ballot_w64(p) != 0ull; }
+__device__ __forceinline__ bool wall(bool p) { return __builtin_amdgcn_ballot_w64(!p) == 0ull; }
+
+__host__ __device__ inline size_t u_lds_rows(uint32_t n_syms) {
+  return (size_t)(kUTabWords + ((n_syms + 3u) & ~3u)) * 4 + (size_t)(kV2Threads / 64) * kUWave + 16;
+}
+__host__ __device__ inline size_t u_lds_prog(uint32_t n_syms) {
+  return u_lds_rows(n_syms) + (size_t)(kV2Threads / 64) * 64 * 12;
+}
+__host__ __device__ inline size_t u_lds(uint32_t n_syms) {
+  return u_lds_prog(n_syms) + (size_t)(kV2Threads / 64) * 4;
+}
+
+template <bool CHARS, int BB, bool HB>
+__global__ __launch_bounds__(kV2Threads) void ku_traverse(UnitDev U, V2Args M) {
+  extern __shared__ __attribute__((aligned(16))) uint8_t smem[];
+  if (M.cursor[1] >= 16ull) return;
+  uint32_t *tabw = reinterpret_cast<uint32_t *>(smem);
+  uint32_t *rlw = tabw + kUTabWords;
+  const uint32_t n_root = (U.n_syms + 3u) & ~3u;
+  for (uint32_t i = threadIdx.x; i < kUTabWords; i += kV2Threads) tabw[i] = U.tables[i];
+  for (uint32_t i = threadIdx.x; i < n_root; i += kV2Threads) rlw[i] = i < U.n_syms ? U.root[i] : 0u;
+  uint32_t *prog = reinterpret_cast<uint32_t *>(smem + u_lds_prog(U.n_syms));
+  if (threadIdx.x < kV2Threads / 64) prog[threadIdx.x] = 0u;
+  __syncthreads();
+  const uint32_t *rl = rlw;
+  const uint4 *t0a = reinterpret_cast<const uint4 *>(tabw + kUT0a);
+  const uint2 *t0b = reinterpret_cast<const uint2 *>(tabw + kUT0b);
+  const uint8_t *tabb = reinterpret_cast<const uint8_t *>(tabw);
+  uint8_t *in_base = smem + (size_t)(kUTabWords + n_root) * 4;
+  const int lane = threadIdx.x & 63, wave = threadIdx.x >> 6;
+  uint8_t *inl = in_base + wave * kUWave + lane * kURow;
+  const uint32_t *row = reinterpret_cast<const uint32_t *>(inl);
+  typedef uint32_t v3u __attribute__((ext_vector_type(3)));
+  const uint32_t wbo = (uint32_t)u_lds_rows(U.n_syms) + (uint32_t)wave * (64u * 12u);
+  const uint2 *slots = U.slots;
+  const int64_t N = (int64_t)M.n_bytes;
+  const uint64_t D = M.n_docs;
+  const int64_t S = (int64_t)M.S;
+  const int rounds = (int)(M.S / kUPiece);
+  const int warm = U.max_len > 1 ? (int)U.max_len - 1 : 0;
+  const int R = (warm + kUPiece - 1) / kUPiece;
+  const uint32_t wave_u = (uint32_t)__builtin_amdgcn_readfirstlane(wave);
+  uint32_t *my_prog = prog + (wave_u & 3u) * 4u + (wave_u >> 2);
+  const uint4 *simd_prog = reinterpret_cast<const uint4 *>(prog + (wave_u & 3u) * 4u);
+  uint32_t n_rounds = 0;
+
+  const uint64_t n_tiles = (M.n_chunks + kV2Threads - 1) / kV2Threads;
+  for (uint64_t tile = blockIdx.x; tile < n_tiles; tile += gridDim.x) {
+    const uint64_t chunk = tile * kV2Threads + threadIdx.x;
+    const uint32_t ev_stride = M.ev_stride;
+    const bool live = chunk < M.n_chunks;
+    const int64_t a = (int64_t)chunk * S;
+    const int64_t e = live ? min(a + S, N) : a;
+    uint64_t dn = 0;
+    int64_t nb = INT64_MAX, doc_start = a, pos = e;
+    uint32_t wfill = 0, wout = 0;
+    const uint64_t wchunk0 = tile * kV2Threads + (uint64_t)wave * 64;
+    uint32_t *wreg = M.evg + wchunk0 * M.ev_stride * 3;
+    const uint32_t wcap = (uint32_t)min<uint64_t>(64, M.n_chunks > wchunk0 ? M.n_chunks - wchunk0 : 0) * M.ev_stride;
+    uint32_t hits = 0;
+    uint32_t lead_total = 0;
+    uint32_t lc = 0, lc_exact = 0;
+    uint32_t E = 0, seq = 0;
+    uint32_t pc = 0;
+    uint4 q1 = make_uint4(0, 0, 0, 0), q2 = q1, q3 = q1;
+    uint32_t w[13] = {0, 0, 0, 0, 0, 0, 0, 0, 0, 0, 0, 0, 0};
+    if (live) {
+      dn = first_boundary(M.doc_off, D, (uint64_t)a);
+      nb = (int64_t)M.doc_off[dn];
+      pos = a;
+      if (nb != a) {
+        doc_start = (int64_t)M.doc_off[dn - 1];
+        pos = a - min<int64_t>(a - doc_start, warm);
+        if (CHARS) M.chunk_doc0[chunk] = (uint32_t)(dn - 1);
+      } else if (CHARS) {
+        M.chunk_doc0[chunk] = (uint32_t)dn;
+      }
+    }
+
+    for (int r = -((R + 3) / 4) * 4 - 2; r <= rounds; r++) {
+      {
+        n_rounds++;
+        if (lane == 0) *my_prog = n_rounds;
+        const uint4 pm = *simd_prog;
+        const uint32_t ahead = ((uint32_t)__builtin_amdgcn_readfirstlane(pm.x) > n_rounds) + ((uint32_t)__builtin_amdgcn_readfirstlane(pm.y) > n_rounds) +
+                               ((uint32_t)__builtin_amdgcn_readfirstlane(pm.z) > n_rounds) + ((uint32_t)__builtin_amdgcn_readfirstlane(pm.w) > n_rounds);
+        if (ahead == 0u)
+          __builtin_amdgcn_s_setprio(0);
+        else if (ahead == 1u)
+          __builtin_amdgcn_s_setprio(1);
+        else if (ahead == 2u)
+          __builtin_amdgcn_s_setprio(2);
+        else
+          __builtin_amdgcn_s_setprio(3);
+      }
+      const int64_t pb = a + (int64_t)r * kUPiece;
+      const int64_t pl = pb + 2 * kUPiece;
+      const int64_t pend = min(pb + kUWin, e);
+      {
+        uint4 v;
+        if ((pl & 63) == 0) {
+          v = load16(M.text, pl, N);
+          q1 = load16(M.text, pl + 16, N);
+          q2 = load16(M.text, pl + 32, N);
+          q3 = load16(M.text, pl + 48, N);
+        } else {
+          v = q1;
+          q1 = q2;
+          q2 = q3;
+        }
+#pragma unroll
+        for (int i = 0; i < 9; i++) w[i] = w[i + 4];
+        w[9] = v.x;
+        w[10] = v.y;
+        w[11] = v.z;
+        w[12] = v.w;
+        uint32_t *dst = reinterpret_cast<uint32_t *>(inl);
+#pragma unroll
+        for (int i = 0; i < 13; i++) dst[i] = w[i];
+      }
+      const bool need = live && pos < pend;
+      if (!wany(need)) continue;
+      uint32_t rel = kURow, lim = 0;
+      if (need) {
+        rel = (uint32_t)(pos - pb + 4);
+        lim = (uint32_t)(pend - pb + 4);
+      }
+      uint32_t nb_rel = (nb >= pb - 4 && nb <= pb + kUWin) ? (uint32_t)(nb - pb + 4) : ~0u;
+      const uint32_t n_rel = (N - pb) <= (int64_t)kUWin ? (uint32_t)max<int64_t>(N - pb + 4, 0) : ~0u;
+      const int32_t a_rel = (int32_t)max<int64_t>(a - pb + 4, -128);
+      const int32_t e_rel = (int32_t)min<int64_t>(e - pb + 4, 128);
+      int32_t docrel = (int32_t)(pb - 4 - doc_start);
+
+      for (;;) {
+        const bool bnd = rel < lim && rel == nb_rel;
+        if (wany(bnd)) {
+          if (bnd) {
+            const int64_t here = pb - 4 + rel;
+            do {
+              M.doc_ev_rank[dn] = seq;
+              M.doc_hit_rank[dn] = hits;
+              if (CHARS) M.doc_lead_rank[dn] = lead_total;
+              dn++;
+              nb = dn <= D ? (int64_t)M.doc_off[dn] : INT64_MAX;
+            } while (nb == here);
+            asm volatile("" : "+v"(nb));
+            nb_rel = (nb <= pb + kUWin) ? (uint32_t)(nb - pb + 4) : ~0u;
+            E = 0;
+            pc = 0;
+            lc = 0;
+            lc_exact = 1;
+            doc_start = here;
+            docrel = -(int32_t)rel;
+          }
+        }
+        uint32_t lim2 = min(lim, nb_rel);
+        const uint32_t dend = min(nb_rel, n_rel);
+        auto decode = [&](uint32_t at, uint32_t &o_code, uint32_t &o_L, bool &o_later) {
+          const uint32_t lo = row[at >> 2], hi = row[(at >> 2) + 1];
+          const uint32_t w4 = __builtin_amdgcn_alignbyte(hi, lo, at & 3u);
+          const uint32_t b0 = w4 & 0xFFu;
+          const uint4 q0 = t0a[b0];
+          const uint2 q1 = t0b[b0];
+          const uint32_t s1 = *reinterpret_cast<const uint32_t *>(tabb + q0.x + ((w4 >> 6) & 0x3FCu));
+          const uint32_t s2 = *reinterpret_cast<const uint32_t *>(tabb + q0.y + ((w4 >> 14) & 0x3FCu));
+          const uint32_t sum = q0.z + s1 + s2;
+          const uint32_t want = q1.y;
+          const bool in_doc = at + want <= dend;
+          o_later = in_doc & at + want > (uint32_t)kURow;
+          const bool whole = in_doc & sum < kUPoison;
+          const bool o_good = whole & (sum - q0.w) < q1.x;
+          o_L = whole ? want : 1u;
+          if (CHARS) o_L |= (b0 & 0xC0u) != 0x80u ? 0x100u : 0u;
+          o_code = o_good ? sum - kUBias : 0u;
+        };
+        uint32_t code, L;
+        {
+          bool later;
+          decode(min(rel, (uint32_t)kURow), code, L, later);
+          lim2 = later ? min(lim2, rel) : lim2;
+          lim = later ? min(lim, rel) : lim;
+        }
+        bool all_left = false;
+        for (;;) {
+          const bool act = rel < lim2;
+          all_left = wall(rel >= (uint32_t)(4 + kUPiece) || rel >= lim);
+          if (all_left || !wany(act)) break;
+          auto trip = [&]() -> uint32_t {
+            uint32_t evc = 0;
+            const bool good = code != 0u;
+            const uint32_t Bq = u_child(E, BB);
+            const bool hdr = u_hdr_pending(E);
+            const bool grp = Bq >= U.big_lo & code >= U.n_low & !hdr;
+            uint32_t se = grp ? (code >> 5) + U.g0 : code;
+            se = hdr ? 0u : se;
+            const uint32_t fc = BB == 23 ? min(code & 7u, 6u) : (code & 7u);
+            const uint32_t Ef = BB == 21 ? E : (E | 0x20000000u);
+            const bool probe = act & good & ((Ef >> ((uint32_t)BB + fc)) & 1u) != 0u & Bq != 0u;
+            unsigned long long enw = 0;
+            uint32_t hdw = 0;
+            {
+              const uint2 *ap = slots + (probe ? (Bq ^ se) : 0u);
+              asm volatile("global_load_dwordx2 %0, %1, off" : "=v"(enw) : "v"(ap) : "memory");
+              if (HB) {
+                const uint2 *hp = slots + ((act & u_nfr(E) & !u_f1(E)) ? Bq : 0u);
+                asm volatile("global_load_dword %0, %1, off" : "=v"(hdw) : "v"(hp) : "memory");
+              }
+            }
+            if (act) {
+              uint32_t n_code, n_L;
+              bool n_later;
+              const uint32_t Lb = CHARS ? (L & 0xFFu) : L;
+              uint32_t rel_adv = rel + Lb;
+              decode(rel_adv, n_code, n_L, n_later);
+              const uint32_t rt = rl[code];
+              const uint32_t rf = rl[pc];
+              const bool viaroot0 = !u_nfr(E) | !good;
+              const bool own0 = viaroot0 | u_f1(E);
+              const uint32_t ft0 = u_f1(E) ? (rf & 0x7FFFFFFFu) : (Bq | u_all_filter(BB) | 0x20000000u);
+              uint32_t miss0 = viaroot0 ? rt : (HB ? (rf & 0x7FFFFFFFu) : ft0);
+              const uint32_t cb = code & 31u;
+              uint32_t lowm = ~(~0u << cb);
+              uint32_t gbit = (grp & probe) ? (1u << cb) : 0u;
+              const bool pg = probe & !grp;
+              const bool pgh = pg & !hdr;
+              const int32_t last = (int32_t)rel_adv - 1;
+              uint32_t wm = (last >= a_rel & last < e_rel) ? ~0u : 0u;
+              uint32_t isl0 = (CHARS && (int32_t)rel >= a_rel) ? (L >> 8) : 0u;
+              if (CHARS) asm volatile("" : "+v"(isl0));
+              if (HB)
+                asm volatile("s_waitcnt vmcnt(0)" : "+v"(enw), "+v"(hdw), "+v"(miss0), "+v"(rel_adv), "+v"(lowm), "+v"(gbit), "+v"(wm), "+v"(n_code), "+v"(n_L) : : "memory");
+              else
+                asm volatile("s_waitcnt vmcnt(0)" : "+v"(enw), "+v"(miss0), "+v"(rel_adv), "+v"(lowm), "+v"(gbit), "+v"(wm), "+v"(n_code), "+v"(n_L) : : "memory");
+              const uint32_t enx = (uint32_t)enw, eny = (uint32_t)(enw >> 32);
+              const bool symeq = u_sym(eny) == se;
+              const bool symhit = symeq & pg;
+              const bool hit = symeq & pgh;
+              const bool redir = (enx & gbit) != 0u;
+              const uint32_t rE = (__builtin_popcount(enx & lowm) + eny ^ code) | u_all_filter(BB);
+              const bool viaroot = !(symhit | redir) & viaroot0;
+              uint32_t missE = HB ? (own0 ? miss0 : hdw) : miss0;
+              missE = redir ? rE : missE;
+              E = symhit ? enx : missE;
+              const bool consumed = hit | viaroot;
+              const bool end = consumed & u_end(E);
+              const uint32_t c4 = hit ? u_c4(eny) : 1u;
+              pc = consumed ? code : pc;
+              if (CHARS) {
+                const uint32_t isl = consumed ? isl0 : 0u;
+                lc += isl;
+                lead_total += isl;
+              }
+              rel = consumed ? rel_adv : rel;
+              const bool park = consumed & n_later;
+              lim2 = park ? rel : lim2;
+              lim = park ? rel : lim;
+              code = consumed ? n_code : code;
+              L = consumed ? n_L : L;
+              evc = end ? (c4 & wm) : 0u;
+            }
+            return evc;
+          };
+          const uint32_t evc = trip();
+          const uint64_t evm = wballot(evc != 0u);
+          if (evm) {
+            const bool ev = evc != 0u;
+            const uint32_t kp = __popcll(evm);
+            if (wfill + kp > 64u) {
+              const uint32_t *q = reinterpret_cast<const uint32_t *>(smem + (wbo + __umul24((uint32_t)lane, 12u)));
+              const v3u r = {q[0], q[1], q[2]};
+              if ((uint32_t)lane < wfill && wout + (uint32_t)lane < wcap) *reinterpret_cast<v3u *>(wreg + (size_t)(wout + lane) * 3) = r;
+              wout += wfill;
+              wfill = 0;
+            }
+            const uint32_t my = wfill + __builtin_amdgcn_mbcnt_hi((uint32_t)(evm >> 32), __builtin_amdgcn_mbcnt_lo((uint32_t)evm, 0u));
+            const uint32_t rx = u_rec_x(u_child(E, BB), (uint32_t)lane, evc, BB), rz = u_rec_z(hits, evc, BB);
+            const uint32_t ry = CHARS ? ((lc << 1) | lc_exact) : (uint32_t)(docrel + (int32_t)rel);
+            if (ev) {
+              uint32_t *d = reinterpret_cast<uint32_t *>(smem + (wbo + __umul24(my, 12u)));
+              d[0] = rx;
+              d[1] = ry;
+              d[2] = rz;
+            }
+            wfill += kp;
+            seq += ev ? 1u : 0u;
+            hits += evc;
+          }
+        }
+        if (all_left || !wany(rel < lim)) break;
+      }
+      if (need) pos = pb - 4 + rel;
+    }
+    {
+      const uint32_t *q = reinterpret_cast<const uint32_t *>(smem + (wbo + __umul24((uint32_t)lane, 12u)));
+      const v3u r = {q[0], q[1], q[2]};
+      if ((uint32_t)lane < wfill && wout + (uint32_t)lane < wcap) *reinterpret_cast<v3u *>(wreg + (size_t)(wout + lane) * 3) = r;
+    }
+    if (live) {
+      M.ev_cnt[chunk] = seq;
+      if (seq > ev_stride) M.cursor[1] = 2ull;
+      if (CHARS) M.lead_cnt[chunk] = lead_total;
+      M.chunk_hits[chunk] = hits;
+      if (e == N) {
+        while (dn <= D) {
+          M.doc_ev_rank[dn] = seq;
+          M.doc_hit_rank[dn] = hits;
+          if (CHARS) M.doc_lead_rank[dn] = lead_total;
+          dn++;
+        }
+      }
+    }
+  }
+}
+
+}
+
+}
diff --git a/aha_amd/csrc/unit.cpp b/aha_amd/csrc/unit.cpp
--- a/aha_amd/csrc/unit.cpp
+++ b/aha_amd/csrc/unit.cpp
@@ -18,10 +18,10 @@
 
 }
 
-static void build_unit_bits(const Automaton &a, UnitImage &u, bool force, uint32_t base_bits) {
+static void build_unit_bits(const Automaton &a, UnitImage &u, bool force, uint32_t limit_bits, uint32_t forced, bool opt_in) {
   u = UnitImage();
-  u.base_bits = base_bits;
-  const uint32_t max_slots = 1u << base_bits;
+  u.base_bits = limit_bits;
+  const uint32_t max_slots = 1u << limit_bits;
   const uint32_t S = a.n_states;
   if (a.n_keys == 0 || S < 2) {
     u.why = "no keys";
@@ -114,7 +114,7 @@
   first[S] = (uint32_t)tr.size();
   u.n_states = (uint32_t)ustates.size();
   u.n_trans = (uint32_t)tr.size();
-  if (getenv("AHA_DEBUG")) fprintf(stderr, "aha: unit image: %u states, %u transitions, %u-bit bases\n", u.n_states, u.n_trans, base_bits);
+  if (getenv("AHA_DEBUG")) fprintf(stderr, "aha: unit image: %u states, %u transitions, at most 2^%u slots\n", u.n_states, u.n_trans, limit_bits);
   if ((uint64_t)u.n_states + u.n_states / 8 + 1 > max_slots) {
     u.why = "more states than the bases address";
     return;
@@ -310,6 +310,7 @@
   freec[0]--;
   idfree[0]--;
   uint32_t n_open = 1, n_big = 0, n_bases = 1;
+  uint32_t id_end = 1;
   std::vector<uint32_t> order, bigs;
   for (uint32_t s : ustates) {
     if (s == 0) continue;
@@ -418,6 +419,7 @@
         }
         for (uint32_t j = 0; j < cnt; j++) {
           used.set(t + j);
+          id_end = std::max(id_end, ((t + j) ^ tr[q + j].sym) + 1u);
           if (!isb.get((t + j) ^ tr[q + j].sym)) {
             isb.set((t + j) ^ tr[q + j].sym);
             idfree[t / kBlk]--;
@@ -483,6 +485,10 @@
   const uint32_t n_shared = n_open * kBlk;
   const uint32_t n_slots = ((n_shared + n_big * bb) + kBlk - 1) & ~(kBlk - 1);
   for (uint32_t bi = 0; bi < n_big; bi++) base[bigs[bi]] = n_shared + bi * bb;
+  for (uint32_t s : ustates) id_end = std::max(id_end, base[s] + 1u);
+  const uint32_t base_bits = limit_bits == 23u ? 23u : u_pick_base_bits(n_slots, id_end, opt_in, forced);
+  u.base_bits = base_bits;
+  if (getenv("AHA_DEBUG")) fprintf(stderr, "aha: unit image: %u slots, identities below %u: %u-bit bases\n", n_slots, id_end, base_bits);
 
   auto word = [&](uint32_t st) -> uint32_t {
     uint32_t flt = 0;
@@ -532,12 +538,15 @@
 
 void build_unit(const Automaton &a, UnitImage &u, bool force) {
   const char *bw = getenv("AHA_UNIT_BASE_BITS");
-  if (bw && strcmp(bw, "23") == 0) {
-    build_unit_bits(a, u, force, 23u);
-    return;
-  }
-  build_unit_bits(a, u, force, 22u);
-  if (!u.ok && strstr(u.why, "bases address")) build_unit_bits(a, u, force, 23u);
+  const uint32_t forced = bw && (strcmp(bw, "21") == 0 || strcmp(bw, "22") == 0 || strcmp(bw, "23") == 0) ? (uint32_t)atoi(bw) : 0u;
+  const char *eng = getenv("AHA_ENGINE"), *sk = getenv("AHA_SKIP"), *pr = getenv("AHA_PAIR");
+  const bool opt_in = (eng && (strcmp(eng, "skip") == 0 || strcmp(eng, "pair") == 0)) || (sk && atoi(sk) != 0) || (pr && atoi(pr) != 0);
+  if (forced == 23u) {
+    build_unit_bits(a, u, force, 23u, forced, opt_in);
+    return;
+  }
+  build_unit_bits(a, u, force, 22u, forced, opt_in);
+  if (!u.ok && strstr(u.why, "bases address")) build_unit_bits(a, u, force, 23u, forced, opt_in);
 }
 
 }
diff --git a/aha_amd/csrc/unit.hpp b/aha_amd/csrc/unit.hpp
--- a/aha_amd/csrc/unit.hpp
+++ b/aha_amd/csrc/unit.hpp
@@ -14,8 +14,17 @@
 constexpr uint32_t kUPoison = 1u << 24;
 constexpr uint32_t kUT0a = 0, kUT0b = 1024, kUA1 = 1536, kUA2 = 2304, kUTabWords = 2816;
 
-AHA_HD inline uint32_t u_child(uint32_t lo, uint32_t bb = 22u) { return lo & ((1u << bb) - 1u); }
+AHA_HD inline uint32_t u_child(uint32_t lo, uint32_t bb) { return lo & ((1u << bb) - 1u); }
 AHA_HD inline uint32_t u_all_filter(uint32_t bb) { return ((1u << (29u - bb)) - 1u) << bb; }
+constexpr uint32_t kUBase21MinSlots = 1u << 17;
+AHA_HD inline uint32_t u_pick_base_bits(uint32_t n_slots, uint32_t id_end, bool opt_in, uint32_t forced) {
+  const bool fits21 = n_slots <= (1u << 21) && id_end <= (1u << 21);
+  const bool fits22 = n_slots <= (1u << 22) && id_end <= (1u << 22);
+  if (forced == 23u || !fits22) return 23u;
+  if (opt_in || forced == 22u || !fits21) return 22u;
+  if (forced == 21u) return 21u;
+  return n_slots > kUBase21MinSlots ? 21u : 22u;
+}
 constexpr uint32_t kUMaxC4 = 255u;
 constexpr uint32_t kUFusedMaxChain = 15u;
 AHA_HD inline uint32_t u_rec_x(uint32_t base, uint32_t lane, uint32_t n, uint32_t bb) {
```

New measurement: 502.0 (median of 6 runs). 1.01x the previous value.
